# Axionis47/semantic-search-kd

Measured on AMD Instinct MI355X. Metric: docs embedded/sec + queries/sec@top-10 (1M×384-d corpus), 1→8 MI355X, higher is better.
Workload: dtype bf16 screen + f32 exact; 1 GPU; cosine top-10: 10000 queries x 1000000 x 384-d fp32 corpus in HBM (configs[1] search), row-sharded over 1 GPU(s), all-gather + merge; corpus_rows=1000000, queries=10000, k=10, queries_per_block=160, corpus_passes=63, slices=4, exact_fallback_queries=0, index_bytes=1536000000, sidecar_bytes=768004096, workspace_bytes=693437184

## Files before the change

### include/sskd_amd.h

```cpp
#ifndef SSKD_AMD_H
#define SSKD_AMD_H

#include <stddef.h>
#include <stdint.h>

#ifdef __cplusplus
extern "C" {
#endif

#define SSKD_ABI_VERSION 1

#define SSKD_OK 0
#define SSKD_ERR_INVALID 1
#define SSKD_ERR_WORKSPACE 2
#define SSKD_ERR_HIP 3
#define SSKD_ERR_UNSUPPORTED 4

#define SSKD_DIM 384
#define SSKD_TILE_ROWS 32
#define SSKD_K_PASS 32
#define SSKD_K_MAX 1024

int sskd_abi_version(void);
const char* sskd_last_error(void);
int sskd_device_count(void);

int64_t sskd_index_padded_rows(int64_t n_rows);
size_t sskd_index_tiled_bytes(int64_t n_rows);

int sskd_index_add_rows(const float* d_rows, int64_t n_rows, int normalize,
                        float* d_tiled, int64_t dst_row0, void* stream);

int sskd_index_get_rows(const float* d_tiled, int64_t row0, int64_t n_rows,
                        float* d_rows, void* stream);

int sskd_l2_normalize_rows(float* d_x, int64_t n_rows, int dim, void* stream);

size_t sskd_index_search_workspace_bytes(int64_t n_rows, int nq, int k);
int sskd_index_search(const float* d_tiled, int64_t n_rows,
                      const float* d_queries, int nq, int k, int64_t id_offset,
                      float* d_out_scores, int64_t* d_out_ids,
                      void* d_workspace, size_t workspace_bytes, void* stream);

typedef struct sskd_search_tuning {
  int32_t queries_per_block;
  int32_t target_workgroups;
  int32_t pruning_pools;
} sskd_search_tuning;

size_t sskd_index_search_workspace_bytes_ex(int64_t n_rows, int nq, int k,
                                            const sskd_search_tuning* tuning);
int sskd_index_search_ex(const float* d_tiled, int64_t n_rows, const float* d_queries, int nq,
                         int k, int64_t id_offset, float* d_out_scores, int64_t* d_out_ids,
                         void* d_workspace, size_t workspace_bytes, void* stream,
                         const sskd_search_tuning* tuning, void* ev_scan_begin, void* ev_scan_end);

int sskd_index_search_profiled(const float* d_tiled, int64_t n_rows,
                               const float* d_queries, int nq, int k, int64_t id_offset,
                               float* d_out_scores, int64_t* d_out_ids,
                               void* d_workspace, size_t workspace_bytes, void* stream,
                               void* ev_scan_begin, void* ev_scan_end);

size_t sskd_index_bf16_bytes(int64_t n_rows);
int sskd_index_make_bf16(const float* d_tiled, int64_t n_rows, void* d_bf16, void* stream);
size_t sskd_index_search_screened_workspace_bytes(int64_t n_rows, int nq, int k);
int sskd_index_search_screened_plan(int64_t n_rows, int nq, int k, int* queries_per_block, int* corpus_passes,
                                    int* n_slices);
int sskd_index_search_screened(const float* d_tiled, const void* d_bf16, int64_t n_rows, const float* d_queries,
                               int nq, int k, int64_t id_offset, float* d_out_scores, int64_t* d_out_ids,
                               int* d_status, void* d_workspace, size_t workspace_bytes, void* stream,
                               void* ev_scan_begin, void* ev_scan_end);

size_t sskd_index_screen_band_scratch_bytes(int nq);
int sskd_index_screen_band(const void* d_bf16, int64_t n_rows, const float* d_queries, int nq, float* d_eps2_out,
                           void* d_scratch, size_t scratch_bytes, void* stream);

int sskd_index_search_screened_plan_claims(int64_t n_rows, int nq, int k, int* claims);
int sskd_index_search_screened_claim(const float* d_tiled, const void* d_bf16, int64_t n_rows, const float* d_queries,
                                     int nq, int k, int64_t id_offset, const uint32_t* d_row_mask, int claim,
                                     float* d_out_scores, int64_t* d_out_ids, int* d_status, void* d_workspace,
                                     size_t workspace_bytes, void* stream, void* ev_scan_begin, void* ev_scan_end);

size_t sskd_index_search_onepass_workspace_bytes(int64_t n_rows, int nq, int k);
int sskd_index_search_onepass(const float* d_tiled, int64_t n_rows, const float* d_queries, int nq,
                              int k, int64_t id_offset, float* d_out_scores, int64_t* d_out_ids,
                              int* d_inexact, void* d_workspace, size_t workspace_bytes,
                              void* stream);

int64_t sskd_row_mask_words(int64_t n_rows);
int sskd_row_mask_pack(const uint8_t* d_flags, int64_t n_rows, uint32_t* d_mask, void* stream);
int sskd_row_mask_update(uint32_t* d_mask, int64_t n_rows, const int64_t* d_rows, int64_t n_ids, int allow,
                         int* d_bad, void* stream);
int sskd_row_mask_and(const uint32_t* d_a, const uint32_t* d_b, int64_t n_rows, uint32_t* d_out, void* stream);
int sskd_row_mask_count(const uint32_t* d_mask, int64_t n_rows, int64_t* d_count, void* stream);

int sskd_index_search_filtered(const float* d_tiled, int64_t n_rows, const float* d_queries, int nq, int k,
                               int64_t id_offset, const uint32_t* d_row_mask, float* d_out_scores,
                               int64_t* d_out_ids, void* d_workspace, size_t workspace_bytes, void* stream,
                               const sskd_search_tuning* tuning, void* ev_scan_begin, void* ev_scan_end);
int sskd_index_search_screened_filtered(const float* d_tiled, const void* d_bf16, int64_t n_rows, const float* d_queries,
                                        int nq, int k, int64_t id_offset, const uint32_t* d_row_mask, float* d_out_scores,
                                        int64_t* d_out_ids, int* d_status, void* d_workspace, size_t workspace_bytes,
                                        void* stream, void* ev_scan_begin, void* ev_scan_end);
int sskd_index_search_onepass_filtered(const float* d_tiled, int64_t n_rows, const float* d_queries, int nq,
                                       int k, int64_t id_offset, const uint32_t* d_row_mask, float* d_out_scores,
                                       int64_t* d_out_ids, int* d_inexact, void* d_workspace,
                                       size_t workspace_bytes, void* stream);

size_t sskd_index_range_search_workspace_bytes(int64_t n_rows, int nq, int64_t max_results);
int sskd_index_range_search(const float* d_tiled, int64_t n_rows, const float* d_queries, int nq,
                            const float* d_thresholds, int64_t id_offset, const uint32_t* d_row_mask, int64_t* d_lims,
                            float* d_out_scores, int64_t* d_out_ids, int64_t max_results, void* d_workspace,
                            size_t workspace_bytes, void* stream);

size_t sskd_range_record_bytes(int nq, int64_t cap);
size_t sskd_range_merge_workspace_bytes(int n_runs, int nq, int64_t max_results);
int sskd_range_merge_packed(const void* d_records, int n_runs, int nq, int64_t cap, int64_t* d_lims,
                            float* d_out_scores, int64_t* d_out_ids, int64_t max_results, void* d_workspace,
                            size_t workspace_bytes, void* stream);

size_t sskd_index_search_grouped_workspace_bytes(int64_t n_rows, int nq, int k, int k_rows);
int sskd_index_search_grouped(const float* d_tiled, int64_t n_rows, const float* d_queries, int nq, int k, int k_rows,
                              int64_t id_offset, const uint32_t* d_row_mask, const int32_t* d_row_group,
                              float* d_out_scores, int64_t* d_out_ids, int32_t* d_out_groups, int32_t* d_out_count,
                              int32_t* d_unproved, int32_t* d_n_unproved, void* d_workspace, size_t workspace_bytes,
                              void* stream);

int sskd_row_mask_rank(const uint32_t* d_mask, int64_t n_rows, int64_t* d_word_prefix, void* stream);
int sskd_index_compact_rows(const float* d_src_tiled, int64_t n_rows, const uint32_t* d_mask,
                            const int64_t* d_word_prefix, float* d_dst_tiled, void* stream);

int sskd_index_mine_select(const float* d_tiled, int64_t n_rows, const float* d_queries, int nq,
                           const float* d_rank_scores, const int64_t* d_rank_ids, int search_k,
                           const int64_t* d_pos_lims, const int32_t* d_pos_rows, const int32_t* d_row_groups,
                           double margin, int top_k, int64_t id_offset, float* d_out_scores, int64_t* d_out_ids,
                           int32_t* d_out_counts, float* d_out_max_pos, void* stream);

size_t sskd_bm25_search_workspace_bytes(int64_t n_rows, int nq, int k);
int sskd_bm25_search_plan(int64_t n_rows, int nq, int k, int* tile_rows, int* tiles, int* queries_per_chunk);
int sskd_bm25_search(const int64_t* d_term_offsets, const int32_t* d_post_rows, const double* d_post_w,
                     const double* d_idf, int64_t n_rows, int64_t n_terms, const int64_t* d_q_lims,
                     const int32_t* d_q_terms, int nq, int k, double* d_out_scores, int64_t* d_out_ids,
                     void* d_workspace, size_t workspace_bytes, void* stream);

int sskd_hybrid_fuse(const float* d_tiled, int64_t n_rows, const float* d_queries, const float* d_dense_scores,
                     const int64_t* d_dense_ids, int kd, const int64_t* d_term_offsets, const int32_t* d_post_rows,
                     const double* d_post_w, const double* d_idf, int64_t n_terms, const int64_t* d_q_lims,
                     const int32_t* d_q_terms, const double* d_bm25_scores, const int64_t* d_bm25_ids, int kb,
                     const uint32_t* d_mask, int method, double w_semantic, double w_bm25, double rrf_k, int nq, int k,
                     int64_t id_offset, double* d_out_scores, int64_t* d_out_ids, int32_t* d_out_counts,
                     float* d_out_dense, double* d_out_bm25, void* stream);

int sskd_eval_judge(const int64_t* d_rank_ids, int nq, int k_rank, int64_t id_offset, const int64_t* d_rel_lims,
                    const int32_t* d_rel_rows, const int32_t* d_rel_grades, int64_t n_rel, const double* d_discounts,
                    const int32_t* cutoffs, int n_cut, int ideal_mode, double* d_out_metrics, void* stream);
int sskd_eval_lists(const float* d_queries, const float* d_docs, int dim, const float* d_scores_in,
                    const int64_t* d_doc_lims, int64_t total, const int32_t* d_grades, const float* d_ref_scores,
                    const double* d_discounts, const int32_t* cutoffs, int n_cut, int ideal_mode, int nq,
                    double* d_out_metrics, float* d_out_scores, int32_t* d_out_order, int64_t* d_out_discordant,
                    void* stream);

int sskd_ivf_search_plan(int nq, int nprobe, int k, int64_t n_rows, int64_t max_list_rows, int* parts, int* chunk_rows,
                         int* workgroups);
size_t sskd_ivf_search_workspace_bytes(int nq, int nprobe, int k, int64_t n_rows, int64_t max_list_rows);
int sskd_ivf_search(const float* d_tiled, int64_t n_rows, const float* d_queries, int nq, const int64_t* d_probe,
                    int nprobe, const int64_t* d_list_offsets, const int32_t* d_list_rows, int nlist, int k,
                    int64_t id_offset, const uint32_t* d_row_mask, float* d_out_scores, int64_t* d_out_ids,
                    void* d_workspace, size_t workspace_bytes, void* stream);
int sskd_ivf_list_sums(const float* d_tiled, int64_t n_rows, const int64_t* d_list_offsets, const int32_t* d_list_rows,
                       int nlist, double* d_sums, void* stream);

int sskd_pq_encode(const float* d_rows, int64_t n, const float* d_centroids, const int64_t* d_assign, int nlist,
                   const float* d_codebooks, int m, uint8_t* d_codes, void* stream);
int sskd_pq_code_sums(const float* d_rows, int64_t n, const float* d_centroids, const int64_t* d_assign, int nlist,
                      const int64_t* d_group_offsets, const int32_t* d_group_rows, int m, double* d_sums,
                      int64_t* d_counts, void* stream);
int sskd_pq_lut(const float* d_queries, int nq, const float* d_codebooks, int m, float* d_lut, void* stream);
int sskd_pq_search_plan(int nq, int nprobe, int k, int refine, int m, int64_t n_rows, int64_t max_list_rows, int* parts,
                        int* min_part_rows, int* workgroups, size_t* lut_bytes);
size_t sskd_pq_search_workspace_bytes(int nq, int nprobe, int k, int refine, int m, int64_t n_rows,
                                      int64_t max_list_rows);
int sskd_pq_search(const float* d_tiled, int64_t n_rows, const float* d_queries, int nq, const int64_t* d_probe,
                   const float* d_probe_scores, int nprobe, const int64_t* d_list_offsets, const int32_t* d_list_rows,
                   int nlist, const uint8_t* d_codes_csr, const float* d_codebooks, int m, int k, int refine,
                   int64_t id_offset, const uint32_t* d_row_mask, float* d_out_scores, int64_t* d_out_ids,
                   int64_t* d_out_candidates, void* d_workspace, size_t workspace_bytes, void* stream);

int sskd_graph_prune(const int32_t* d_knn, int64_t n_rows, int knn_k, int M, int32_t* d_fwd, void* stream);
int sskd_graph_merge(const int32_t* d_fwd, const int32_t* d_rev, int64_t n_rows, int M, int32_t* d_graph, void* stream);
int sskd_graph_search_plan(int nq, int k, int ef, int width, int M, int n_seeds, int* workgroups, int* threads,
                           int* lds_bytes, int* step_rows);
size_t sskd_graph_search_workspace_bytes(int nq, int k, int ef, int width, int M, int n_seeds);
int sskd_graph_search(const float* d_tiled, int64_t n_rows, const int32_t* d_graph, int M, const float* d_queries, int nq,
                      const int64_t* d_seeds, int n_seeds, const int32_t* d_seed_rows, int64_t n_seed_rows, int k, int ef,
                      int width, int max_iterations, int64_t id_offset, const uint32_t* d_row_mask, float* d_out_scores,
                      int64_t* d_out_ids, int32_t* d_out_iterations, void* stream);

#define SSKD_LATE_TQ_MAX 128
#define SSKD_LATE_R_MAX 1024
int sskd_late_pack_tokens(const void* d_hidden, const int32_t* d_lengths, const int64_t* d_offsets, int B, int S,
                          int64_t n_tokens, void* d_tokens, void* stream);
int sskd_late_rerank_plan(int nq, int max_tq, int R, int k, int* workgroups, int* threads, int* lds_bytes, int* chunk);
size_t sskd_late_rerank_workspace_bytes(int nq, int R);
int sskd_late_rerank(const void* d_q_tokens, const int64_t* q_lims, const int64_t* d_q_lims, int nq, const void* d_tokens,
                     const int64_t* d_tok_lims, int64_t n_rows, int64_t n_tokens, const int64_t* d_candidates, int R, int k,
                     int64_t id_offset, float* d_out_scores, int64_t* d_out_ids, float* d_out_raw, void* d_workspace,
                     size_t workspace_bytes, void* stream);

#define SSKD_LATE_C_MAX 65536
int sskd_latec_compress(const void* d_tokens, const int64_t* d_assign, int64_t n, const void* d_centroids, int C,
                       const float* d_cutoffs, const float* d_weights, int nbits, int32_t* d_cid, float* d_scale,
                       uint8_t* d_codes, int64_t row0, int64_t n_store, void* stream);
int sskd_latec_rerank_plan(int nq, int max_tq, int R, int k, int nbits, int* workgroups, int* threads, int* lds_bytes,
                                     int* chunk);
size_t sskd_latec_rerank_workspace_bytes(int nq, int R);
int sskd_latec_rerank(const void* d_q_tokens, const int64_t* q_lims, const int64_t* d_q_lims, int nq,
                                const int32_t* d_cid, const float* d_scale, const uint8_t* d_codes, int nbits,
                                const void* d_centroids, int C, const float* d_weights, const int64_t* d_tok_lims, int64_t n_rows,
                                int64_t n_tokens, const int64_t* d_candidates, int R, int k, int64_t id_offset,
                                float* d_out_scores, int64_t* d_out_ids, float* d_out_raw, void* d_workspace,
                                size_t workspace_bytes, void* stream);

int sskd_kd_loss(const float* d_student, const float* d_teacher, int batch, int n_docs,
                 float temperature, float contrastive_temperature, float w_margin_mse,
                 float w_listwise, float w_contrastive, float* d_losses, float* d_grad,
                 float* d_row_workspace, void* stream);

int sskd_index_search_plan(int64_t n_rows, int nq, int k, int* queries_per_block,
                           int* corpus_passes, int* n_slices, int* waves_per_block,
                           int* scan_passes);

int sskd_index_search_plan_ex(int64_t n_rows, int nq, int k, const sskd_search_tuning* tuning,
                              int* queries_per_block, int* corpus_passes, int* n_slices,
                              int* waves_per_block, int* scan_passes);

int sskd_topk_merge(const float* d_scores, const int64_t* d_ids, int n_lists, int nq,
                    int k_in, int k_out, float* d_out_scores, int64_t* d_out_ids,
                    void* stream);

size_t sskd_topk_record_bytes(int nq, int k);
int sskd_topk_merge_packed(const void* d_records, int n_lists, int nq, int k_in, int k_out,
                           float* d_out_scores, int64_t* d_out_ids, void* stream);

int sskd_similarity(const float* d_q, int nq, const float* d_d, int nd, int dim,
                    float* d_out, void* stream);


int sskd_pool_normalize(const void* d_hidden, int hidden_is_bf16, const int32_t* d_mask,
                        int B, int S, int normalize, float* d_out, void* stream);

typedef struct sskd_encoder_config {
  int32_t vocab_size;
  int32_t hidden;
  int32_t layers;
  int32_t heads;
  int32_t intermediate;
  int32_t max_positions;
  int32_t type_vocab;
  float layer_norm_eps;
} sskd_encoder_config;

typedef struct sskd_encoder_layer_weights {
  const void* wqkv;
  const float* bqkv;
  const void* wo;
  const float* bo;
  const float* ln1_g;
  const float* ln1_b;
  const void* w1;
  const float* b1;
  const void* w2;
  const float* b2;
  const float* ln2_g;
  const float* ln2_b;
} sskd_encoder_layer_weights;

typedef struct sskd_encoder_weights {
  const void* word_emb;
  const void* pos_emb;
  const void* type_emb;
  const float* emb_ln_g;
  const float* emb_ln_b;
  const sskd_encoder_layer_weights* layers;
} sskd_encoder_weights;

size_t sskd_encoder_workspace_bytes(const sskd_encoder_config* cfg, int B, int S);

int sskd_encoder_forward(const sskd_encoder_config* cfg, const sskd_encoder_weights* w,
                         const int32_t* d_ids, const int32_t* d_mask, int B, int S,
                         int normalize, float* d_out, void* d_workspace,
                         size_t workspace_bytes, void* stream);

int sskd_encoder_hidden(const sskd_encoder_config* cfg, const sskd_encoder_weights* w,
                        const int32_t* d_ids, const int32_t* d_mask, int B, int S,
                        void* d_hidden_bf16, void* d_workspace, size_t workspace_bytes,
                        void* stream);

int sskd_encoder_probe(const sskd_encoder_config* cfg, const sskd_encoder_weights* w,
                       const int32_t* d_ids, const int32_t* d_mask, const int32_t* d_seg, int B, int S,
                       void* d_hidden_bf16, void* d_context_bf16, void* d_workspace,
                       size_t workspace_bytes, void* stream);


int sskd_pack_plan(const int32_t* lengths, int n_seq, int capacity, int32_t* table, int* n_rows);

int sskd_pack_tokens(const int32_t* d_flat_ids, const int32_t* d_cu_seqlens, const int32_t* d_table,
                     int n_seq, int n_rows, int capacity, int32_t* d_ids, int32_t* d_seg, void* stream);

int sskd_encoder_forward_packed(const sskd_encoder_config* cfg, const sskd_encoder_weights* w,
                                const int32_t* d_ids, const int32_t* d_seg, int n_rows, int capacity,
                                const int32_t* d_table, int n_seq, int normalize, float* d_out,
                                void* d_workspace, size_t workspace_bytes, void* stream);

typedef struct sskd_generic_config {
  int32_t vocab_size;
  int32_t hidden;
  int32_t layers;
  int32_t heads;
  int32_t intermediate;
  int32_t max_positions;
  int32_t type_vocab;
  float layer_norm_eps;
  int32_t pos_offset;
} sskd_generic_config;

typedef struct sskd_generic_layer_weights {
  const void* wqkv;
  const void* wqkv_t;
  const void* wo;
  const void* wo_t;
  const void* w1;
  const void* w1_t;
  const void* w2;
  const void* w2_t;
  const float* bqkv;
  const float* bo;
  const float* ln1_g;
  const float* ln1_b;
  const float* b1;
  const float* b2;
  const float* ln2_g;
  const float* ln2_b;
} sskd_generic_layer_weights;

typedef struct sskd_generic_weights {
  const void* word_emb;
  const void* pos_emb;
  const void* type_emb;
  const float* emb_ln_g;
  const float* emb_ln_b;
  const sskd_generic_layer_weights* layers;
} sskd_generic_weights;

typedef struct sskd_generic_layer_grads {
  float* wqkv;
  float* bqkv;
  float* wo;
  float* bo;
  float* ln1_g;
  float* ln1_b;
  float* w1;
  float* b1;
  float* w2;
  float* b2;
  float* ln2_g;
  float* ln2_b;
} sskd_generic_layer_grads;

typedef struct sskd_generic_grads {
  float* word_emb;
  float* pos_emb;
  float* type_emb;
  float* emb_ln_g;
  float* emb_ln_b;
  const sskd_generic_layer_grads* layers;
} sskd_generic_grads;

size_t sskd_generic_workspace_bytes(const sskd_generic_config* cfg, int B, int S, int training);

int sskd_generic_forward(const sskd_generic_config* cfg, const sskd_generic_weights* w, const int32_t* d_ids,
                         const int32_t* d_mask, int B, int S, int training, int pool, int normalize, void* d_out,
                         void* d_workspace, size_t workspace_bytes, void* stream);

int sskd_generic_backward(const sskd_generic_config* cfg, const sskd_generic_weights* w, const sskd_generic_grads* grads,
                          const int32_t* d_ids, const int32_t* d_mask, int B, int S, int normalize, const float* d_dout,
                          void* d_workspace, size_t workspace_bytes, void* stream);

size_t sskd_teacher_workspace_bytes(const sskd_generic_config* cfg, int B, int S);
int sskd_teacher_score(const sskd_generic_config* cfg, const sskd_generic_weights* w, const float* d_head_dense_w,
                       const float* d_head_dense_b, const float* d_head_out_w, const float* d_head_out_b,
                       const int32_t* d_ids, const int32_t* d_mask, int B, int S, float* d_logits, void* d_workspace,
                       size_t workspace_bytes, void* stream);

int sskd_gemm_nt_bf16(const void* d_a, const void* d_b, void* d_c, const float* d_bias, int M, int N, int K,
                      int c_is_f32, int accumulate, void* stream);
int sskd_gemm_backend(int mode);
int sskd_gemm_tn_bf16(const void* d_a, const void* d_b, float* d_c, int64_t T, int M, int N, void* stream);

typedef struct sskd_gemm_desc {
  const void* a;
  const void* b;
  void* c;
  const float* bias;
  int64_t lda, ldb, ldc;
  int64_t sa1, sa2, sb1, sb2, sc1, sc2;
  int32_t m, n, k;
  int32_t batch1, batch2;
  float alpha;
  int32_t c_is_f32;
  int32_t accumulate;
  int32_t split_k;
  int32_t act;
} sskd_gemm_desc;

int sskd_gemm_nt_ex(const sskd_gemm_desc* d, void* stream);

enum {
  SSKD_OP_ATTENTION_FWD = 1,
  SSKD_OP_ATTENTION_BWD = 2,
  SSKD_OP_SOFTMAX_FWD = 3,
  SSKD_OP_SOFTMAX_BWD = 4,
  SSKD_OP_ADD_LN_FWD = 5,
  SSKD_OP_LN_BWD = 6,
  SSKD_OP_GELU_FWD = 7,
  SSKD_OP_GELU_BWD = 8,
  SSKD_OP_GELU_BWD_COLSUM = 9,
  SSKD_OP_COLSUM = 10,
  SSKD_OP_ADD = 11,
  SSKD_OP_TRANSPOSE = 12,
  SSKD_OP_EMBED_FWD = 13,
  SSKD_OP_EMBED_BWD = 14,
  SSKD_OP_POOL_FWD = 15,
  SSKD_OP_POOL_BWD = 16,
  SSKD_OP_GEMM_TN = 17
};
int sskd_generic_op(int op, const void* const* ptrs, int n_ptrs, const int64_t* ints, int n_ints, const float* floats,
                    int n_floats, void* stream);


int sskd_tokenizer_create(const char* vocab_blob, int64_t blob_bytes, void** handle);
void sskd_tokenizer_destroy(void* handle);

int sskd_tokenizer_encode(void* handle, const char* text_blob, const int64_t* offsets, int n_texts,
                          int max_len, int n_threads, int32_t* out_ids, int64_t out_capacity,
                          int32_t* out_lengths, uint8_t* out_needs_unicode, int64_t* out_total);

#ifdef __cplusplus
}
#endif
#endif
```

### semantic-search-kd_amd/_native.py

```python
from __future__ import annotations

import ctypes as C
from pathlib import Path
from typing import Optional

_LIB_PATH = Path(__file__).resolve().parent / "libsskd_amd.so"

SSKD_OK = 0
SSKD_DIM = 384
SSKD_TILE_ROWS = 32
SSKD_K_PASS = 32
SSKD_K_MAX = 1024

_ERR_NAMES = {1: "INVALID", 2: "WORKSPACE", 3: "HIP", 4: "UNSUPPORTED"}


class NativeError(RuntimeError):

    def __init__(self, code: int, message: str):
        super().__init__(f"sskd_amd[{_ERR_NAMES.get(code, code)}]: {message}")
        self.code = code


class EncoderConfig(C.Structure):
    _fields_ = [
        ("vocab_size", C.c_int32),
        ("hidden", C.c_int32),
        ("layers", C.c_int32),
        ("heads", C.c_int32),
        ("intermediate", C.c_int32),
        ("max_positions", C.c_int32),
        ("type_vocab", C.c_int32),
        ("layer_norm_eps", C.c_float),
    ]


class EncoderLayerWeights(C.Structure):
    _fields_ = [
        (n, C.c_void_p)
        for n in ("wqkv", "bqkv", "wo", "bo", "ln1_g", "ln1_b", "w1", "b1", "w2", "b2", "ln2_g", "ln2_b")
    ]


class EncoderWeights(C.Structure):
    _fields_ = [
        ("word_emb", C.c_void_p),
        ("pos_emb", C.c_void_p),
        ("type_emb", C.c_void_p),
        ("emb_ln_g", C.c_void_p),
        ("emb_ln_b", C.c_void_p),
        ("layers", C.POINTER(EncoderLayerWeights)),
    ]


class GenericConfig(C.Structure):
    _fields_ = [
        ("vocab_size", C.c_int32), ("hidden", C.c_int32), ("layers", C.c_int32), ("heads", C.c_int32),
        ("intermediate", C.c_int32), ("max_positions", C.c_int32), ("type_vocab", C.c_int32),
        ("layer_norm_eps", C.c_float), ("pos_offset", C.c_int32),
    ]


GENERIC_LAYER_W = ("wqkv", "wqkv_t", "wo", "wo_t", "w1", "w1_t", "w2", "w2_t",
                   "bqkv", "bo", "ln1_g", "ln1_b", "b1", "b2", "ln2_g", "ln2_b")
GENERIC_LAYER_G = ("wqkv", "bqkv", "wo", "bo", "ln1_g", "ln1_b", "w1", "b1", "w2", "b2", "ln2_g", "ln2_b")


class GenericLayerWeights(C.Structure):
    _fields_ = [(n, C.c_void_p) for n in GENERIC_LAYER_W]


class GenericWeights(C.Structure):
    _fields_ = [(n, C.c_void_p) for n in ("word_emb", "pos_emb", "type_emb", "emb_ln_g", "emb_ln_b")] + [
        ("layers", C.POINTER(GenericLayerWeights))
    ]


class GenericLayerGrads(C.Structure):
    _fields_ = [(n, C.c_void_p) for n in GENERIC_LAYER_G]


class GenericGrads(C.Structure):
    _fields_ = [(n, C.c_void_p) for n in ("word_emb", "pos_emb", "type_emb", "emb_ln_g", "emb_ln_b")] + [
        ("layers", C.POINTER(GenericLayerGrads))
    ]


class GemmDesc(C.Structure):

    _fields_ = [("a", C.c_void_p), ("b", C.c_void_p), ("c", C.c_void_p), ("bias", C.c_void_p)] + [
        (n, C.c_int64) for n in ("lda", "ldb", "ldc", "sa1", "sa2", "sb1", "sb2", "sc1", "sc2")
    ] + [(n, C.c_int32) for n in ("m", "n", "k", "batch1", "batch2")] + [("alpha", C.c_float)] + [
        (n, C.c_int32) for n in ("c_is_f32", "accumulate", "split_k", "act")
    ]


OP_ATTENTION_FWD, OP_ATTENTION_BWD, OP_SOFTMAX_FWD, OP_SOFTMAX_BWD, OP_ADD_LN_FWD, OP_LN_BWD = 1, 2, 3, 4, 5, 6
OP_GELU_FWD, OP_GELU_BWD, OP_GELU_BWD_COLSUM, OP_COLSUM, OP_ADD, OP_TRANSPOSE = 7, 8, 9, 10, 11, 12
OP_EMBED_FWD, OP_EMBED_BWD, OP_POOL_FWD, OP_POOL_BWD, OP_GEMM_TN = 13, 14, 15, 16, 17


class SearchTuning(C.Structure):

    _fields_ = [("queries_per_block", C.c_int32), ("target_workgroups", C.c_int32), ("pruning_pools", C.c_int32)]


_vp, _i, _i64, _sz = C.c_void_p, C.c_int, C.c_int64, C.c_size_t
_ip = C.POINTER(C.c_int)
_f = C.c_float
SIGNATURES = {
    "sskd_abi_version": (_i, []),
    "sskd_last_error": (C.c_char_p, []),
    "sskd_device_count": (_i, []),
    "sskd_index_padded_rows": (_i64, [_i64]),
    "sskd_index_tiled_bytes": (_sz, [_i64]),
    "sskd_index_add_rows": (_i, [_vp, _i64, _i, _vp, _i64, _vp]),
    "sskd_index_get_rows": (_i, [_vp, _i64, _i64, _vp, _vp]),
    "sskd_l2_normalize_rows": (_i, [_vp, _i64, _i, _vp]),
    "sskd_index_search_workspace_bytes": (_sz, [_i64, _i, _i]),
    "sskd_index_search": (_i, [_vp, _i64, _vp, _i, _i, _i64, _vp, _vp, _vp, _sz, _vp]),
    "sskd_index_search_profiled": (_i, [_vp, _i64, _vp, _i, _i, _i64, _vp, _vp, _vp, _sz, _vp, _vp, _vp]),
    "sskd_index_search_plan": (_i, [_i64, _i, _i, _ip, _ip, _ip, _ip, _ip]),
    "sskd_index_search_workspace_bytes_ex": (_sz, [_i64, _i, _i, C.POINTER(SearchTuning)]),
    "sskd_index_search_ex": (
        _i, [_vp, _i64, _vp, _i, _i, _i64, _vp, _vp, _vp, _sz, _vp, C.POINTER(SearchTuning), _vp, _vp]
    ),
    "sskd_index_search_plan_ex": (_i, [_i64, _i, _i, C.POINTER(SearchTuning), _ip, _ip, _ip, _ip, _ip]),
    "sskd_topk_record_bytes": (_sz, [_i, _i]),
    "sskd_topk_merge_packed": (_i, [_vp, _i, _i, _i, _i, _vp, _vp, _vp]),
    "sskd_index_bf16_bytes": (_sz, [_i64]),
    "sskd_index_make_bf16": (_i, [_vp, _i64, _vp, _vp]),
    "sskd_index_search_screened_workspace_bytes": (_sz, [_i64, _i, _i]),
    "sskd_index_search_screened_plan": (_i, [_i64, _i, _i, _ip, _ip, _ip]),
    "sskd_index_search_screened": (_i, [_vp, _vp, _i64, _vp, _i, _i, _i64, _vp, _vp, _vp, _vp, _sz, _vp, _vp, _vp]),
    "sskd_index_search_screened_plan_claims": (_i, [_i64, _i, _i, _ip]),
    "sskd_index_search_screened_claim": (
        _i, [_vp, _vp, _i64, _vp, _i, _i, _i64, _vp, _i, _vp, _vp, _vp, _vp, _sz, _vp, _vp, _vp]
    ),
    "sskd_index_screen_band_scratch_bytes": (_sz, [_i]),
    "sskd_index_screen_band": (_i, [_vp, _i64, _vp, _i, _vp, _vp, _sz, _vp]),
    "sskd_index_search_onepass_workspace_bytes": (_sz, [_i64, _i, _i]),
    "sskd_index_search_onepass": (_i, [_vp, _i64, _vp, _i, _i, _i64, _vp, _vp, _vp, _vp, _sz, _vp]),
    "sskd_row_mask_words": (_i64, [_i64]),
    "sskd_row_mask_pack": (_i, [_vp, _i64, _vp, _vp]),
    "sskd_row_mask_update": (_i, [_vp, _i64, _vp, _i64, _i, _vp, _vp]),
    "sskd_row_mask_and": (_i, [_vp, _vp, _i64, _vp, _vp]),
    "sskd_row_mask_count": (_i, [_vp, _i64, _vp, _vp]),
    "sskd_index_search_filtered": (
        _i, [_vp, _i64, _vp, _i, _i, _i64, _vp, _vp, _vp, _vp, _sz, _vp, C.POINTER(SearchTuning), _vp, _vp]
    ),
    "sskd_index_search_screened_filtered": (
        _i, [_vp, _vp, _i64, _vp, _i, _i, _i64, _vp, _vp, _vp, _vp, _vp, _sz, _vp, _vp, _vp]
    ),
    "sskd_index_search_onepass_filtered": (_i, [_vp, _i64, _vp, _i, _i, _i64, _vp, _vp, _vp, _vp, _vp, _sz, _vp]),
    "sskd_index_range_search_workspace_bytes": (_sz, [_i64, _i, _i64]),
    "sskd_index_range_search": (_i, [_vp, _i64, _vp, _i, _vp, _i64, _vp, _vp, _vp, _vp, _i64, _vp, _sz, _vp]),
    "sskd_range_record_bytes": (_sz, [_i, _i64]),
    "sskd_range_merge_workspace_bytes": (_sz, [_i, _i, _i64]),
    "sskd_range_merge_packed": (_i, [_vp, _i, _i, _i64, _vp, _vp, _vp, _i64, _vp, _sz, _vp]),
    "sskd_index_search_grouped_workspace_bytes": (_sz, [_i64, _i, _i, _i]),
    "sskd_index_search_grouped": (
        _i, [_vp, _i64, _vp, _i, _i, _i, _i64, _vp, _vp, _vp, _vp, _vp, _vp, _vp, _vp, _vp, _sz, _vp]
    ),
    "sskd_row_mask_rank": (_i, [_vp, _i64, _vp, _vp]),
    "sskd_index_compact_rows": (_i, [_vp, _i64, _vp, _vp, _vp, _vp]),
    "sskd_index_mine_select": (
        _i, [_vp, _i64, _vp, _i, _vp, _vp, _i, _vp, _vp, _vp, C.c_double, _i, _i64, _vp, _vp, _vp, _vp, _vp]
    ),
    "sskd_bm25_search_workspace_bytes": (_sz, [_i64, _i, _i]),
    "sskd_bm25_search_plan": (_i, [_i64, _i, _i, _ip, _ip, _ip]),
    "sskd_bm25_search": (_i, [_vp, _vp, _vp, _vp, _i64, _i64, _vp, _vp, _i, _i, _vp, _vp, _vp, _sz, _vp]),
    "sskd_hybrid_fuse": (
        _i, [_vp, _i64, _vp, _vp, _vp, _i, _vp, _vp, _vp, _vp, _i64, _vp, _vp, _vp, _vp, _i, _vp, _i, C.c_double,
             C.c_double, C.c_double, _i, _i, _i64, _vp, _vp, _vp, _vp, _vp, _vp]
    ),
    "sskd_eval_judge": (_i, [_vp, _i, _i, _i64, _vp, _vp, _vp, _i64, _vp, _vp, _i, _i, _vp, _vp]),
    "sskd_eval_lists": (
        _i, [_vp, _vp, _i, _vp, _vp, _i64, _vp, _vp, _vp, _vp, _i, _i, _i, _vp, _vp, _vp, _vp, _vp]
    ),
    "sskd_ivf_search_plan": (_i, [_i, _i, _i, _i64, _i64, _ip, _ip, _ip]),
    "sskd_ivf_search_workspace_bytes": (_sz, [_i, _i, _i, _i64, _i64]),
    "sskd_ivf_search": (_i, [_vp, _i64, _vp, _i, _vp, _i, _vp, _vp, _i, _i, _i64, _vp, _vp, _vp, _vp, _sz, _vp]),
    "sskd_ivf_list_sums": (_i, [_vp, _i64, _vp, _vp, _i, _vp, _vp]),
    "sskd_pq_encode": (_i, [_vp, _i64, _vp, _vp, _i, _vp, _i, _vp, _vp]),
    "sskd_pq_code_sums": (_i, [_vp, _i64, _vp, _vp, _i, _vp, _vp, _i, _vp, _vp, _vp]),
    "sskd_pq_lut": (_i, [_vp, _i, _vp, _i, _vp, _vp]),
    "sskd_pq_search_plan": (_i, [_i, _i, _i, _i, _i, _i64, _i64, _ip, _ip, _ip, C.POINTER(_sz)]),
    "sskd_pq_search_workspace_bytes": (_sz, [_i, _i, _i, _i, _i, _i64, _i64]),
    "sskd_pq_search": (
        _i, [_vp, _i64, _vp, _i, _vp, _vp, _i, _vp, _vp, _i, _vp, _vp, _i, _i, _i, _i64, _vp, _vp, _vp, _vp, _vp, _sz, _vp]
    ),
    "sskd_graph_prune": (_i, [_vp, _i64, _i, _i, _vp, _vp]),
    "sskd_graph_merge": (_i, [_vp, _vp, _i64, _i, _vp, _vp]),
    "sskd_graph_search_plan": (_i, [_i, _i, _i, _i, _i, _i, _ip, _ip, _ip, _ip]),
    "sskd_graph_search_workspace_bytes": (_sz, [_i, _i, _i, _i, _i, _i]),
    "sskd_graph_search": (
        _i, [_vp, _i64, _vp, _i, _vp, _i, _vp, _i, _vp, _i64, _i, _i, _i, _i, _i64, _vp, _vp, _vp, _vp, _vp]
    ),
    "sskd_late_pack_tokens": (_i, [_vp, _vp, _vp, _i, _i, _i64, _vp, _vp]),
    "sskd_late_rerank_plan": (_i, [_i, _i, _i, _i, _ip, _ip, _ip, _ip]),
    "sskd_late_rerank_workspace_bytes": (_sz, [_i, _i]),
    "sskd_late_rerank": (
        _i, [_vp, _vp, _vp, _i, _vp, _vp, _i64, _i64, _vp, _i, _i, _i64, _vp, _vp, _vp, _vp, _sz, _vp]
    ),
    "sskd_latec_compress": (_i, [_vp, _vp, _i64, _vp, _i, _vp, _vp, _i, _vp, _vp, _vp, _i64, _i64, _vp]),
    "sskd_latec_rerank_plan": (_i, [_i, _i, _i, _i, _i, _ip, _ip, _ip, _ip]),
    "sskd_latec_rerank_workspace_bytes": (_sz, [_i, _i]),
    "sskd_latec_rerank": (
        _i, [_vp, _vp, _vp, _i, _vp, _vp, _vp, _i, _vp, _i, _vp, _vp, _i64, _i64, _vp, _i, _i, _i64, _vp, _vp, _vp, _vp, _sz, _vp]
    ),
    "sskd_topk_merge": (_i, [_vp, _vp, _i, _i, _i, _i, _vp, _vp, _vp]),
    "sskd_kd_loss": (_i, [_vp, _vp, _i, _i, _f, _f, _f, _f, _f, _vp, _vp, _vp, _vp]),
    "sskd_similarity": (_i, [_vp, _i, _vp, _i, _i, _vp, _vp]),
    "sskd_pool_normalize": (_i, [_vp, _i, _vp, _i, _i, _i, _vp, _vp]),
    "sskd_encoder_workspace_bytes": (_sz, [C.POINTER(EncoderConfig), _i, _i]),
    "sskd_encoder_forward": (
        _i,
        [C.POINTER(EncoderConfig), C.POINTER(EncoderWeights), _vp, _vp, _i, _i, _i, _vp, _vp, _sz, _vp],
    ),
    "sskd_pack_plan": (_i, [_vp, _i, _i, _vp, _ip]),
    "sskd_pack_tokens": (_i, [_vp, _vp, _vp, _i, _i, _i, _vp, _vp, _vp]),
    "sskd_encoder_forward_packed": (
        _i,
        [C.POINTER(EncoderConfig), C.POINTER(EncoderWeights), _vp, _vp, _i, _i, _vp, _i, _i, _vp, _vp, _sz, _vp],
    ),
    "sskd_generic_workspace_bytes": (_sz, [C.POINTER(GenericConfig), _i, _i, _i]),
    "sskd_generic_forward": (
        _i, [C.POINTER(GenericConfig), C.POINTER(GenericWeights), _vp, _vp, _i, _i, _i, _i, _i, _vp, _vp, _sz, _vp]
    ),
    "sskd_generic_backward": (
        _i, [C.POINTER(GenericConfig), C.POINTER(GenericWeights), C.POINTER(GenericGrads), _vp, _vp, _i, _i, _i, _vp,
             _vp, _sz, _vp]
    ),
    "sskd_teacher_workspace_bytes": (_sz, [C.POINTER(GenericConfig), _i, _i]),
    "sskd_teacher_score": (
        _i, [C.POINTER(GenericConfig), C.POINTER(GenericWeights), _vp, _vp, _vp, _vp, _vp, _vp, _i, _i, _vp, _vp, _sz, _vp]
    ),
    "sskd_gemm_nt_bf16": (_i, [_vp, _vp, _vp, _vp, _i, _i, _i, _i, _i, _vp]),
    "sskd_gemm_backend": (_i, [_i]),
    "sskd_gemm_tn_bf16": (_i, [_vp, _vp, _vp, _i64, _i, _i, _vp]),
    "sskd_gemm_nt_ex": (_i, [C.POINTER(GemmDesc), _vp]),
    "sskd_generic_op": (_i, [_i, C.POINTER(_vp), _i, C.POINTER(_i64), _i, C.POINTER(_f), _i, _vp]),
    "sskd_tokenizer_create": (_i, [C.c_char_p, _i64, C.POINTER(C.c_void_p)]),
    "sskd_tokenizer_destroy": (None, [_vp]),
    "sskd_tokenizer_encode": (_i, [_vp, C.c_char_p, _vp, _i, _i, _i, _vp, _i64, _vp, _vp, C.POINTER(_i64)]),
    "sskd_encoder_hidden": (
        _i,
        [C.POINTER(EncoderConfig), C.POINTER(EncoderWeights), _vp, _vp, _i, _i, _vp, _vp, _sz, _vp],
    ),
    "sskd_encoder_probe": (
        _i,
        [C.POINTER(EncoderConfig), C.POINTER(EncoderWeights), _vp, _vp, _vp, _i, _i, _vp, _vp, _vp, _sz, _vp],
    ),
}

_lib: Optional[C.CDLL] = None


def lib_path() -> Path:
    return _LIB_PATH


def load() -> C.CDLL:
    global _lib
    if _lib is not None:
        return _lib
    if not _LIB_PATH.exists():
        raise ImportError(
            f"{_LIB_PATH} is missing: the MI355X HIP extension is not built. "
            "Run `python -c 'import __graft_entry__ as g; g.build()'` (needs hipcc). "
            "There is no CPU fallback."
        )
    lib = C.CDLL(str(_LIB_PATH))
    for name, (res, args) in SIGNATURES.items():
        fn = getattr(lib, name)
        fn.restype = res
        fn.argtypes = args
    _lib = lib
    return lib


def check(code: int) -> None:
    if code != SSKD_OK:
        msg = load().sskd_last_error()
        raise NativeError(code, msg.decode("utf-8", "replace") if msg else "unknown error")


def require_gpu() -> None:
    import torch

    if not torch.cuda.is_available():
        raise RuntimeError(
            "semantic-search-kd_amd is an MI355X-only backend: no HIP device is visible "
            "(torch.cuda.is_available() is False) and there is no CPU path."
        )
    load()


def current_stream_ptr(device=None) -> int:
    import torch

    return int(torch.cuda.current_stream(device).cuda_stream)


def grown(buf, need_bytes: int, device):
    import torch

    if buf is not None and buf.numel() >= need_bytes:
        return buf
    return torch.empty(max(int(need_bytes), 1), dtype=torch.uint8, device=device)


def as_device_i32(x, device):
    import numpy as np
    import torch

    t = x if isinstance(x, torch.Tensor) else torch.from_numpy(np.ascontiguousarray(np.asarray(x)))
    return t.to(device=device, dtype=torch.int32)


def padded_ids_mask(input_ids, attention_mask, device, pad_id: int = 0):
    import torch

    ids = as_device_i32(input_ids, device)
    mask = torch.ones_like(ids) if attention_mask is None else as_device_i32(attention_mask, device)
    S = ids.shape[1]
    Sp = max(32, -(-S // 32) * 32)
    if Sp != S:
        ids = torch.nn.functional.pad(ids, (0, Sp - S), value=pad_id)
        mask = torch.nn.functional.pad(mask, (0, Sp - S))
    return ids.contiguous(), mask.contiguous()
```

### semantic-search-kd_amd/csrc/screen.hip

```cpp
#include "search_device.h"
#include "search_host.h"

#include <algorithm>
#include <cfloat>

using sskd::require_shard_rows;

namespace {

typedef __bf16 sbf16x8 __attribute__((ext_vector_type(8)));
constexpr int BSTEPS = DIM / 16;
constexpr int BTILE_VEC = BSTEPS * 64;
#ifndef SSKD_SCREEN_BGROUP
#define SSKD_SCREEN_BGROUP 6
#endif
#ifndef SSKD_SCREEN_WAVES
#define SSKD_SCREEN_WAVES 12
#endif
#ifndef SSKD_SCREEN_RING
#define SSKD_SCREEN_RING 2
#endif
constexpr int BGROUP = SSKD_SCREEN_BGROUP;
constexpr int SCREEN_RING = SSKD_SCREEN_RING;
constexpr int BGROUP_Q5 = 3, SCREEN_RING_Q5 = 2;
#ifndef SSKD_SCREEN_TAU_REFRESH_TILES
#define SSKD_SCREEN_TAU_REFRESH_TILES 64
#endif
constexpr int SCREEN_TAU_REFRESH_TILES = SSKD_SCREEN_TAU_REFRESH_TILES;
constexpr int SCREEN_WAVES = SSKD_SCREEN_WAVES;
template <int BG, int RG>
struct ScreenRingOk {
  static_assert(BSTEPS % BG == 0 && (BSTEPS / BG) % RG == 0 && RG >= 2, "screening prefetch geometry");
  static constexpr bool value = true;
};
static_assert(ScreenRingOk<BGROUP, SCREEN_RING>::value && ScreenRingOk<BGROUP_Q5, SCREEN_RING_Q5>::value, "");
constexpr float SCREEN_ACC_SLACK = 1.0e-4f;
constexpr int SCREEN_MAX_CAND = 256;
constexpr int SCREEN_FALLBACK_TIER1 = 1024;
constexpr int SCREEN_LIGHT_MAX_TILES_PER_WAVE = 330;
constexpr int SCREEN_CUS = 256;

__global__ __launch_bounds__(256) void tile_colsum_kernel(const float4* __restrict__ tiled, int64_t n_tiles,
                                                          float* __restrict__ colsum) {
  const int c = threadIdx.x % CHUNKS, g = threadIdx.x / CHUNKS;
  if (g >= 2) return;
  float4 a = make_float4(0.f, 0.f, 0.f, 0.f);
  for (int64_t t = blockIdx.x; t < n_tiles; t += gridDim.x) {
    const float4* src = tiled + t * (int64_t)(TILE_ROWS * CHUNKS);
#pragma unroll 4
    for (int r = g; r < TILE_ROWS; r += 2) {
      const float4 v = src[r * CHUNKS + c];
      a.x += v.x; a.y += v.y; a.z += v.z; a.w += v.w;
    }
  }
  atomicAdd(colsum + 4 * c + 0, a.x); atomicAdd(colsum + 4 * c + 1, a.y);
  atomicAdd(colsum + 4 * c + 2, a.z); atomicAdd(colsum + 4 * c + 3, a.w);
}

constexpr int SIDECAR_NORM_BYTES = 4096;
constexpr int SIDECAR_ABSMAX_WORD = 3;
constexpr int SIDECAR_COLSUM_OFF = 64;

__global__ __launch_bounds__(256) void make_bf16_tiles_kernel(const float4* __restrict__ tiled, int64_t n_tiles, int64_t n_rows,
                                                              sbf16x8* __restrict__ out, int* __restrict__ norm_block) {
  __shared__ float rowss[3][32];
  __shared__ float mu[DIM];
  __shared__ int amax;
  const int64_t t = blockIdx.x;
  if (threadIdx.x < 96) rowss[threadIdx.x >> 5][threadIdx.x & 31] = 0.f;
  if (threadIdx.x == 0) amax = 0;
  const float inv_n = 1.0f / (float)n_rows;
  for (int c = threadIdx.x; c < DIM; c += 256) mu[c] = reinterpret_cast<const float*>(norm_block)[SIDECAR_COLSUM_OFF + c] * inv_n;
  __syncthreads();
  const float4* src = tiled + t * (int64_t)(TILE_ROWS * CHUNKS);
  for (int v = threadIdx.x; v < BTILE_VEC; v += 256) {
    const int sidx = v >> 6, l = v & 63, r = l & 31, hh = l >> 5;
    const int u = 2 * sidx + hh;
    const float4 a = src[tile_idx4(r, 2 * u)], b = src[tile_idx4(r, 2 * u + 1)];
    const float x[8] = {a.x, a.y, a.z, a.w, b.x, b.y, b.z, b.w};
    const bool live = t * TILE_ROWS + r < n_rows;
    sbf16x8 o;
    float nn = 0.f, bb = 0.f, dd = 0.f;
    int am = 0;
#pragma unroll
    for (int e = 0; e < 8; ++e) {
      const float xc = live ? x[e] - mu[8 * u + e] : 0.f;
      o[e] = (__bf16)xc;
      const float xr = (float)o[e];
      const float d = xr - xc;
      am = max(am, __float_as_int(x[e]) & 0x7fffffff);
      nn = fmaf(x[e], x[e], nn);
      bb = fmaf(xr, xr, bb);
      dd = fmaf(d, d, dd);
    }
    out[t * BTILE_VEC + v] = o;
    atomicAdd(&rowss[0][r], nn);
    atomicAdd(&rowss[1][r], bb);
    atomicAdd(&rowss[2][r], dd);
    atomicMax(&amax, am);
  }
  __syncthreads();
  if (threadIdx.x < 96) {
    const float v = rowss[threadIdx.x >> 5][threadIdx.x & 31];
    atomicMax(norm_block + (threadIdx.x >> 5), __float_as_int(v < INFINITY ? v : INFINITY));
  }
  if (threadIdx.x == 96) atomicMax(norm_block + SIDECAR_ABSMAX_WORD, amax);
}

constexpr float SCREEN_MIN_CORPUS = 0x1p-40f, SCREEN_MIN_QUERY = 0x1p-96f;
constexpr float SCREEN_MIN_BAND = 0x1p-100f, SCREEN_MAX_BAND = 0x1p+100f;
__global__ __launch_bounds__(256) void screen_setup_kernel(const float* __restrict__ queries, int nq,
                                                           const int* __restrict__ max_norm2, float* __restrict__ eps2,
                                                           int* __restrict__ tau, int* __restrict__ fb_count,
                                                           int* __restrict__ d_status, int* __restrict__ cursors,
                                                           int n_cursors) {
  for (int i = blockIdx.x * 256 + threadIdx.x; i < n_cursors; i += gridDim.x * 256) cursors[i] = 0;
  if (threadIdx.x < 44) {
    const int64_t i = (int64_t)blockIdx.x * 44 + threadIdx.x;
    if (i < (int64_t)nq * 11) tau[i] = (int)0x80000000;
  }
  if (blockIdx.x == 0) {
    if (threadIdx.x < 64) fb_count[threadIdx.x] = 0;
    if (threadIdx.x < 2) d_status[threadIdx.x] = 0;
  }
  const int lane = threadIdx.x & 63;
  const int q = blockIdx.x * 4 + (threadIdx.x >> 6);
  if (q >= nq) return;
  float xs[DIM / 64];
  int am = 0;
#pragma unroll
  for (int i = 0; i < DIM / 64; ++i) {
    xs[i] = queries[(int64_t)q * DIM + lane + 64 * i];
    am = max(am, __float_as_int(xs[i]) & 0x7fffffff);
  }
#pragma unroll
  for (int o = 32; o > 0; o >>= 1) am = max(am, __shfl_xor(am, o));
  const int ex = min(max(am >> 23, 1), 253);
  const float down = __int_as_float(ex << 23), up = __int_as_float((254 - ex) << 23);
  float ss = 0.f, dd = 0.f;
#pragma unroll
  for (int i = 0; i < DIM / 64; ++i) {
    const float x = xs[i];
    const float d = ((float)(__bf16)x - x) * up;
    const float xu = x * up;
    ss = fmaf(xu, xu, ss);
    dd = fmaf(d, d, dd);
  }
  ss = wave_sum(ss);
  dd = wave_sum(dd);
  if (lane == 0) {
    const float cn = sqrtf(__int_as_float(max_norm2[0])), cb = sqrtf(__int_as_float(max_norm2[1])),
                cd = sqrtf(__int_as_float(max_norm2[2]));
    const float ca = __int_as_float(max_norm2[SIDECAR_ABSMAX_WORD]), qa = __int_as_float(am);
    const float qn = sqrtf(ss), qd = sqrtf(dd);
    const float band = 2.0f * (qd * cb + qn * cd + SCREEN_ACC_SLACK * qn * fmaxf(cn, cb)) * 1.0002f * down;
    const bool zero = (qa == 0.f || ca == 0.f) && band == 0.f;
    const bool sound = zero || (qa >= SCREEN_MIN_QUERY && ca >= SCREEN_MIN_CORPUS && ca < INFINITY &&
                                band >= SCREEN_MIN_BAND && band <= SCREEN_MAX_BAND);
    eps2[q] = sound ? band + 1e-30f : INFINITY;
  }
}

template <int BG>
__device__ __forceinline__ void load_bgroup(sbf16x8 (&buf)[BG], const sbf16x8* __restrict__ base, unsigned lane_off) {
  asm volatile("" : "+v"(lane_off));
#pragma unroll
  for (int s = 0; s < BG; ++s)
    buf[s] = *reinterpret_cast<const sbf16x8*>(reinterpret_cast<const char*>(base + s * 64) + lane_off);
}

typedef __attribute__((address_space(3))) const sbf16x8 screen_lds_frag;
constexpr int SCREEN_FRAGS_PER_BASE = 64;
template <int QB>
constexpr int screen_frag_bases() { return (QB * BSTEPS + SCREEN_FRAGS_PER_BASE - 1) / SCREEN_FRAGS_PER_BASE; }
#ifndef SSKD_SCREEN_FRAG_DEPTH
#define SSKD_SCREEN_FRAG_DEPTH 2
#endif
constexpr int SCREEN_FRAG_DEPTH = SSKD_SCREEN_FRAG_DEPTH;
static_assert(SCREEN_FRAG_DEPTH >= 2, "the fragment ring holds the MFMA's own operand and at least one read ahead");

template <int QB, int NB>
__device__ __forceinline__ sbf16x8 read_qfrag(screen_lds_frag* const (&qbase)[NB], int I) {
  const int f = (I % QB) * BSTEPS + I / QB;
  return qbase[f / SCREEN_FRAGS_PER_BASE][(f % SCREEN_FRAGS_PER_BASE) * 64];
}

template <int QB, int G, int BG, int D, int NB>
__device__ __forceinline__ void compute_bgroup(const sbf16x8 (&a)[BG], screen_lds_frag* const (&qbase)[NB], sbf16x8 (&b)[D],
                                               f32x16 (&acc)[QB]) {
  constexpr int N = BG * QB, I0 = G * N, TOTAL = BSTEPS * QB;
  asm volatile("" ::: "memory");
#ifndef SSKD_SCREEN_ABL_NOLDS
  if constexpr (G == 0) {
#pragma unroll
    for (int i = 0; i < D - 1; ++i) b[i % D] = read_qfrag<QB>(qbase, i);
  }
#endif
#pragma unroll
  for (int i = 0; i < N; ++i) {
    const int I = I0 + i, s = i / QB, qq = i % QB;
#ifdef SSKD_SCREEN_ABL_NOLDS
    const sbf16x8 bi = a[(s + qq) % BG];
#else
    if (I + D - 1 < TOTAL) b[(I + D - 1) % D] = read_qfrag<QB>(qbase, I + D - 1);
    const sbf16x8 bi = b[I % D];
#endif
    __builtin_amdgcn_sched_barrier(0);
    acc[qq] = __builtin_amdgcn_mfma_f32_32x32x16_bf16(a[s], bi, acc[qq], 0, 0, 0);
    __builtin_amdgcn_sched_barrier(0);
  }
}

template <int QB, int G, int BG, int RG, int D, int NB>
__device__ __forceinline__ void screen_tile_groups(sbf16x8 (&buf)[RG][BG], const sbf16x8* __restrict__ tile,
                                                   screen_lds_frag* const (&qbase)[NB], sbf16x8 (&b)[D], f32x16 (&acc)[QB],
                                                   bool more, int64_t next_tile, unsigned lane_off) {
  constexpr int NG = BSTEPS / BG;
  if constexpr (G < NG) {
    constexpr int PG = G + RG - 1;
#ifndef SSKD_SCREEN_ABL_NOGLOBAL
    if constexpr (PG < NG) load_bgroup<BG>(buf[PG % RG], tile + PG * BG * 64, lane_off);
    else if (more) load_bgroup<BG>(buf[PG % RG], tile + next_tile + (PG - NG) * BG * 64, lane_off);
#endif
    compute_bgroup<QB, G, BG, D, NB>(buf[G % RG], qbase, b, acc);
    screen_tile_groups<QB, G + 1, BG, RG, D, NB>(buf, tile, qbase, b, acc, more, next_tile, lane_off);
  }
}

#ifndef SSKD_SCREEN_CAP
#define SSKD_SCREEN_CAP 64
#endif
#ifndef SSKD_SCREEN_FIN_ENTRIES
#define SSKD_SCREEN_FIN_ENTRIES 640
#endif
constexpr int SCREEN_CAP = SSKD_SCREEN_CAP;
#ifndef SSKD_SCREEN_PRE_TILES
#define SSKD_SCREEN_PRE_TILES 64
#endif
constexpr int SCREEN_PRE_TILES = SSKD_SCREEN_PRE_TILES;
constexpr int SCREEN_FIN_ENTRIES = SSKD_SCREEN_FIN_ENTRIES;
static_assert(SCREEN_FIN_ENTRIES >= 640, "the streaming path of the finalize kernel parks 64 x 10 scores in the stage");

#ifndef SSKD_SCREEN_CLAIM_TILES
#define SSKD_SCREEN_CLAIM_TILES 8
#endif
constexpr int SCREEN_CLAIM_TILES = SSKD_SCREEN_CLAIM_TILES;
#ifndef SSKD_SCREEN_CLAIM_MIN_CHUNKS
#define SSKD_SCREEN_CLAIM_MIN_CHUNKS 2
#endif
#ifndef SSKD_SCREEN_CLAIM_MIN_QBLOCKS
#define SSKD_SCREEN_CLAIM_MIN_QBLOCKS 32
#endif
constexpr int SCREEN_CLAIM_MIN_CHUNKS = SSKD_SCREEN_CLAIM_MIN_CHUNKS, SCREEN_CLAIM_MIN_QBLOCKS = SSKD_SCREEN_CLAIM_MIN_QBLOCKS;
static_assert(SCREEN_CLAIM_TILES >= 2, "the claim for the next chunk is issued one whole tile before the chunk in hand ends");
#ifdef SSKD_SCREEN_NO_STEAL
constexpr bool SCREEN_STEAL = false;
#else
constexpr bool SCREEN_STEAL = true;
#endif

struct ScreenAppendParams {
  const sbf16x8* tiled;
  const float* queries;
  const float* eps2;
  uint2* cand;
  int* cand_cnt;
  int* tau;
  int* gpool;
  int* cursors;
  int64_t n_rows;
  int n_tiles;
  int nq;
  int n_slices;
  int tiles_per_slice;
  int lists_per_query;
  int pre_tiles;
  int pre_tps;
  int claim;
  const uint32_t* row_mask;
#ifdef SSKD_SCREEN_STAMPS
  unsigned long long* stamps;
#endif
};

__device__ __attribute__((noinline)) int screen_compact_run(unsigned long long* run, int n, float thr) {
  int w = 0;
  for (int i = 0; i < n; ++i) {
    const unsigned long long e = __hip_atomic_load(run + i, __ATOMIC_RELAXED, __HIP_MEMORY_SCOPE_AGENT);
    if (__uint_as_float((unsigned)e) >= thr) run[w++] = e;
  }
  return w;
}

template <int K, int QB, int WAVES, bool BOUND_ONLY, bool LIGHT, int BG, int RG, bool MASKED = false>
__device__ __forceinline__ void screen_tiles(const ScreenAppendParams& p, int t_begin, int t_end, int slice, int* cursors,
                                             int wave, int j, int h, int q0,
                                             const sbf16x8* __restrict__ qlane,
                                             int* __restrict__ pool, int* __restrict__ wthr, uint2* run0, int64_t run_stride,
                                             bool ragged, float (&gthr)[QB], const float (&band)[QB], int (&cnt)[QB]) {
  sbf16x8 buf[RG][BG];
  constexpr int NB = screen_frag_bases<QB>();
  screen_lds_frag* qbase[NB];
#pragma unroll
  for (int nb = 0; nb < NB; ++nb) {
    qbase[nb] = (screen_lds_frag*)qlane + nb * SCREEN_FRAGS_PER_BASE * 64;
    asm volatile("" : "+v"(qbase[nb]));
  }
  sbf16x8 qfrag[SCREEN_FRAG_DEPTH];
  const unsigned lane_off = (unsigned)(j + 32 * h) * 16u;
  int n_real = p.nq - q0 - j;
  asm volatile("" : "+v"(n_real));
  constexpr int CH = SCREEN_CLAIM_TILES;
  int t, next_t, c_end = 0, next_end = 0, sl = slice, s_begin = t_begin, s_end = t_end, left = p.n_slices - 1, drawn = 0;
  bool in_flight = false;
  const auto draw = [&]() {
    drawn = 0;
    int at = sl;
    asm volatile("" : "+v"(at));
    if (j + 32 * h == 0) drawn = __hip_atomic_fetch_add(cursors + at, 1, __ATOMIC_RELAXED, __HIP_MEMORY_SCOPE_AGENT);
    in_flight = true;
  };
  const auto drawn_chunk = [&]() -> int {
    for (;;) {
      if (!in_flight) draw();
      in_flight = false;
      const int c = __builtin_amdgcn_readfirstlane(drawn);
      const int nt = s_begin + (c + WAVES) * CH;
      if (nt < s_end) {
        next_end = min(nt + CH, s_end);
        return nt;
      }
      if (!SCREEN_STEAL || left == 0) return -1;
      --left;
      sl = sl + 1 == p.n_slices ? 0 : sl + 1;
      s_begin = sl * p.tiles_per_slice;
      s_end = min(s_begin + p.tiles_per_slice, p.n_tiles);
    }
  };
  const bool dealt = BOUND_ONLY || !p.claim;
  if (dealt) {
    t = t_begin + wave < t_end ? t_begin + wave : -1;
  } else {
    t = t_begin + wave * CH;
    c_end = min(t + CH, t_end);
    if (t >= t_end) {
      t = drawn_chunk();
      c_end = next_end;
    }
  }
  if (t >= 0) {
#pragma unroll
    for (int g = 0; g + 1 < RG; ++g) load_bgroup<BG>(buf[g], p.tiled + (int64_t)t * BTILE_VEC + g * BG * 64, lane_off);
  }

  for (int tiles_done = 0; t >= 0; t = next_t, ++tiles_done) {
    if (dealt) {
      next_t = t + WAVES < t_end ? t + WAVES : -1;
    } else {
      const int rem = c_end - t;
      if (rem == 2) draw();
      next_t = t + 1;
      if (rem == 1) {
        next_t = drawn_chunk();
        c_end = next_end;
      }
    }
    const sbf16x8* tile = p.tiled + (int64_t)t * BTILE_VEC;
    uint32_t mword = 0xFFFFFFFFu;
    if constexpr (MASKED) mword = tile_mask_word(p.row_mask, t);
    const bool exchange = !BOUND_ONLY && (tiles_done == 0 || tiles_done == 16 || tiles_done % SCREEN_TAU_REFRESH_TILES == 0);
#pragma unroll
    for (int qq = 0; qq < QB; ++qq) {
      const int w = wthr[qq * 32 + j];
      gthr[qq] = fmaxf(gthr[qq], ordered_to_float(w) - band[qq]);
      if (exchange && (qq * 32 < n_real))
        gthr[qq] = fmaxf(gthr[qq],
                         ordered_to_float(exchange_bound<K>(p.gpool, p.tau + q0 + qq * 32 + j, q0 + qq * 32 + j, w)) - band[qq]);
    }
    f32x16 acc[QB];
#pragma unroll
    for (int qq = 0; qq < QB; ++qq)
#pragma unroll
      for (int r = 0; r < 16; ++r) acc[qq][r] = 0.f;

    screen_tile_groups<QB, 0, BG, RG, SCREEN_FRAG_DEPTH, NB>(buf, tile, qbase, qfrag, acc, next_t >= 0,
                                                             BOUND_ONLY ? (int64_t)WAVES * BTILE_VEC
                                                                        : (int64_t)(next_t - t) * BTILE_VEC, lane_off);

    const int rowbase = t * TILE_ROWS + 4 * h;
    if (ragged && (int64_t)(t + 1) * TILE_ROWS > p.n_rows) {
#pragma unroll
      for (int qq = 0; qq < QB; ++qq)
#pragma unroll
        for (int r = 0; r < 16; ++r)
          if (rowbase + acc_row(r) >= p.n_rows) acc[qq][r] = -INFINITY;
    }
    if constexpr (MASKED) apply_tile_mask<QB>(acc, mword, h);
#ifdef SSKD_SCREEN_ABL_NOLIST
#pragma unroll
    for (int qq = 0; qq < QB; ++qq)
#pragma unroll
      for (int r = 0; r < 16; ++r) asm volatile("" ::"v"(acc[qq][r]));
    if (false)
#endif
#pragma unroll
    for (int qq = 0; qq < QB; ++qq) {
      float m = acc[qq][0];
#pragma unroll
      for (int r = 1; r < 16; ++r) m = fmaxf(m, acc[qq][r]);
      if constexpr (BOUND_ONLY) {
        if ((qq * 32 < n_real) && m >= gthr[qq]) {
          int xid = rowbase;
#pragma unroll
          for (int r = 15; r >= 0; --r) xid = acc[qq][r] == m ? rowbase + acc_row(r) : xid;
          const int xi = float_to_ordered(m);
          if (pool_offer<K>(pool + (qq * 32 + j) * K, wthr + qq * 32 + j, xi)) {
            int qa = q0 + qq * 32 + j;
            asm volatile("" : "+v"(qa));
            bucket_forward<K>(p.gpool, qa, xid, xi);
          }
          gthr[qq] = fmaxf(gthr[qq], ordered_to_float(wthr[qq * 32 + j]) - band[qq]);
        }
      } else
      if (__any((qq * 32 < n_real) && m >= gthr[qq])) {
#ifndef SSKD_SCREEN_NO_COMPACT
        {
          const bool tight = cnt[qq] > SCREEN_CAP - 16 && cnt[qq] <= SCREEN_CAP;
          if (__any(tight)) {
            __builtin_amdgcn_s_waitcnt(0x0F70);
            if (tight) cnt[qq] = screen_compact_run(reinterpret_cast<unsigned long long*>(run0 + qq * run_stride), cnt[qq], gthr[qq]);
          }
        }
#endif
        bool grew = false;
#pragma unroll
        for (int r = 0; r < 16; ++r) {
          const float x = acc[qq][r];
          const int xid = rowbase + acc_row(r);
          const bool take = (qq * 32 < n_real) && x >= gthr[qq];
          {
            if (take) {
              {
                unsigned long long* const run = reinterpret_cast<unsigned long long*>(run0 + qq * run_stride);
                if (cnt[qq] < SCREEN_CAP)
                  run[cnt[qq]] = (unsigned long long)__float_as_uint(x) | ((unsigned long long)(unsigned)xid << 32);
                ++cnt[qq];
              }
              if (!LIGHT && tiles_done > 0) {
                const int xi = float_to_ordered(x);
                if (pool_offer<K>(pool + (qq * 32 + j) * K, wthr + qq * 32 + j, xi) && (qq * 32 < n_real))
                  bucket_forward<K>(p.gpool, q0 + qq * 32 + j, xid, xi);
              }
              grew = true;
            }
          }
        }
        if (grew) {
          if constexpr (LIGHT) {
            int xid = rowbase;
#pragma unroll
            for (int r = 15; r >= 0; --r) xid = acc[qq][r] == m ? rowbase + acc_row(r) : xid;
            const int xi = float_to_ordered(m);
            if (pool_offer<K>(pool + (qq * 32 + j) * K, wthr + qq * 32 + j, xi) && tiles_done > 0)
              bucket_forward<K>(p.gpool, q0 + qq * 32 + j, xid, xi);
          } else {
            if (tiles_done == 0) pool_offer<K>(pool + (qq * 32 + j) * K, wthr + qq * 32 + j, float_to_ordered(m));
          }
          gthr[qq] = fmaxf(gthr[qq], ordered_to_float(wthr[qq * 32 + j]) - band[qq]);
        }
      }
    }
  }

}

template <int K, int QB, int WAVES, bool LIGHT, int BG, int RG, bool MASKED = false>
__global__ __launch_bounds__(WAVES * 64) void screen_append_kernel(ScreenAppendParams p) {
  extern __shared__ float4 qs_raw[];
  sbf16x8* const qs = reinterpret_cast<sbf16x8*>(qs_raw);
  const int tid = threadIdx.x;
  const int lane = tid & 63;
  const int wave = __builtin_amdgcn_readfirstlane(tid >> 6);
  const int j = lane & 31, h = lane >> 5;
  const int n_qblocks = gridDim.x / p.n_slices;
  const int xcd = blockIdx.x & 7, within = blockIdx.x >> 3;
  const int logical = xcd * (gridDim.x >> 3) + min(xcd, (int)(gridDim.x & 7)) + within;
  const int slice = logical / n_qblocks;
  const int qblk = logical % n_qblocks;
  const int q0 = qblk * (32 * QB);
#ifdef SSKD_SCREEN_STAMPS
  unsigned long long* const stamp = p.stamps + ((int64_t)blockIdx.x * WAVES + wave) * 3;
  if (lane == 0) stamp[0] = __builtin_amdgcn_s_memrealtime();
#endif

  for (int idx = tid; idx < QB * BSTEPS * 64; idx += WAVES * 64) {
    const int l = idx & 63, sidx = (idx >> 6) % BSTEPS, qq = idx / (64 * BSTEPS);
    const int q = q0 + qq * 32 + (l & 31);
    sbf16x8 v;
#pragma unroll
    for (int e = 0; e < 8; ++e) v[e] = (__bf16)0.f;
    if (q < p.nq) {
      const float4* src = reinterpret_cast<const float4*>(p.queries + (int64_t)q * DIM + 16 * sidx + 8 * (l >> 5));
      const float4 a = src[0], b = src[1];
      v[0] = (__bf16)a.x; v[1] = (__bf16)a.y; v[2] = (__bf16)a.z; v[3] = (__bf16)a.w;
      v[4] = (__bf16)b.x; v[5] = (__bf16)b.y; v[6] = (__bf16)b.z; v[7] = (__bf16)b.w;
    }
    qs[idx] = v;
  }
  int* const pool = reinterpret_cast<int*>(qs + QB * BSTEPS * 64);
  int* const wthr = pool + QB * 32 * K;
  for (int i = tid; i < QB * 32 * (K + 1); i += WAVES * 64) pool[i] = (int)0x80000000;
  __syncthreads();
  const sbf16x8* qlane = qs + lane;

  float gthr[QB];
  float band[QB];
  int cnt[QB];
  bool real[QB];
#pragma unroll
  for (int qq = 0; qq < QB; ++qq) {
    gthr[qq] = -FLT_MAX;
    const int qg = q0 + qq * 32 + j;
    real[qq] = qg < p.nq;
    band[qq] = p.eps2[real[qq] ? qg : p.nq - 1];
    cnt[qq] = 0;
  }
  const int my_list = (slice * WAVES + wave) * 2 + h;
  uint2* const run0 = p.cand + ((int64_t)min(q0 + j, p.nq - 1) * p.lists_per_query + my_list) * SCREEN_CAP;
  const int64_t run_stride = (int64_t)32 * p.lists_per_query * SCREEN_CAP;

  const bool ragged = (p.n_rows & 31) != 0;

  const int t_begin = slice * p.tiles_per_slice;
  const int t_end = min(t_begin + p.tiles_per_slice, p.n_tiles);
  if (p.pre_tps > 0) {
    const int s_begin = slice * p.pre_tps;
    const int s_end = min(s_begin + p.pre_tps, p.pre_tiles);
    screen_tiles<K, QB, WAVES, true, LIGHT, BG, RG, MASKED>(p, s_begin, s_end, slice, nullptr, wave, j, h, q0, qlane,
                                             pool, wthr, run0, run_stride, ragged, gthr, band, cnt);
#pragma unroll
    for (int qq = 0; qq < QB; ++qq)
      if (real[qq] && h == 0) atomicMax(p.tau + q0 + qq * 32 + j, wthr[qq * 32 + j]);
    __syncthreads();
    if ((SCREEN_STEAL && p.claim) || (s_begin < t_end && t_begin < s_end)) {
      for (int i = tid; i < QB * 32 * K; i += WAVES * 64) pool[i] = (int)0x80000000;
      __syncthreads();
    }
  }
#ifdef SSKD_SCREEN_STAMPS
  if (lane == 0) stamp[1] = __builtin_amdgcn_s_memrealtime();
#endif
  screen_tiles<K, QB, WAVES, false, LIGHT, BG, RG, MASKED>(p, t_begin, t_end, slice, p.cursors + (int64_t)qblk * p.n_slices,
                                            wave, j, h, q0, qlane, pool, wthr, run0, run_stride, ragged, gthr, band, cnt);
#ifdef SSKD_SCREEN_STAMPS
  if (lane == 0) stamp[2] = __builtin_amdgcn_s_memrealtime();
#endif

  int jt = j;
  asm volatile("" : "+v"(jt));
#pragma unroll
  for (int qq = 0; qq < QB; ++qq) {
    const int q = q0 + qq * 32 + jt;
    if (q < p.nq) p.cand_cnt[(int64_t)q * p.lists_per_query + my_list] = cnt[qq];
  }
}

struct ScreenFinalAppendParams {
  const uint2* cand;
  const int* cand_cnt;
  const float* eps2;
  const float* rows;
  const float* queries;
  int lists, k, nq;
  int64_t id_offset;
  float* out_scores;
  int64_t* out_ids;
  int* fb_count;
  int* fb_qid;
  float* fb_queries;
};

__global__ __launch_bounds__(64) void screen_finalize_append_kernel(ScreenFinalAppendParams p) {
  extern __shared__ __attribute__((aligned(16))) float fin_lds[];
  float* const es = fin_lds;
  int* const ei = reinterpret_cast<int*>(fin_lds + SCREEN_FIN_ENTRIES);
  float* const qv = fin_lds + 2 * SCREEN_FIN_ENTRIES;
  int* const ci = reinterpret_cast<int*>(qv + DIM);
  const int q = blockIdx.x, lane = threadIdx.x;
  for (int c = lane; c < DIM; c += 64) qv[c] = p.queries[(int64_t)q * DIM + c];

  bool bad = !(p.eps2[q] < INFINITY);
  int total = 0;
  for (int l0 = 0; l0 < p.lists; l0 += 64) {
    const int l = l0 + lane;
    const int c = l < p.lists ? p.cand_cnt[(int64_t)q * p.lists + l] : 0;
    if (c > SCREEN_CAP) bad = true;
    total += wave_sum(min(c, SCREEN_CAP));
  }
  int M = 0;
  float tau;
  if (total <= SCREEN_FIN_ENTRIES) {
    int base = 0;
    for (int l0 = 0; l0 < p.lists; l0 += 64) {
      const int l = l0 + lane;
      const int c = l < p.lists ? min(p.cand_cnt[(int64_t)q * p.lists + l], SCREEN_CAP) : 0;
      int incl = c;
#pragma unroll
      for (int o = 1; o < 64; o <<= 1) {
        const int v = __shfl_up(incl, o);
        if (lane >= o) incl += v;
      }
      const int off = base + incl - c;
      const uint2* src = p.cand + ((int64_t)q * p.lists + l) * SCREEN_CAP;
      for (int i = 0; i < c; ++i) {
        const uint2 e = src[i];
        es[off + i] = __uint_as_float(e.x);
        ei[off + i] = (int)e.y;
      }
      base += __shfl(incl, 63);
    }
    const int L = total;
    __builtin_amdgcn_s_waitcnt(0xC07F);

    float bs = INFINITY;
    int bi = -1;
    bool have = false;
    float kth = -INFINITY;
    int found = 0;
    for (int r = 0; r < p.k; ++r) {
      float s = -INFINITY;
      int i = -1;
      for (int e = lane; e < L; e += 64) {
        pick_after(s, i, es[e], ei[e], have, bs, bi);
      }
      wave_argbest(s, i);
      if (i < 0) break;
      bs = s; bi = i; have = true;
      kth = s;
      ++found;
    }
    tau = found == p.k ? kth - p.eps2[q] : -INFINITY;

    for (int e0 = 0; e0 < L; e0 += 64) {
      const int e = e0 + lane;
      const bool in = e < L && es[e] >= tau;
      const unsigned long long mask = __ballot(in);
      if (in) {
        const int slot = M + __popcll(mask & ((1ull << lane) - 1ull));
        if (slot < SCREEN_MAX_CAND) ci[slot] = ei[e];
      }
      M += __popcll(mask);
    }
  } else {
    float top[10];
#pragma unroll
    for (int i = 0; i < 10; ++i) top[i] = -INFINITY;
    for (int l = lane; l < p.lists; l += 64) {
      const int c = min(p.cand_cnt[(int64_t)q * p.lists + l], SCREEN_CAP);
      const uint2* src = p.cand + ((int64_t)q * p.lists + l) * SCREEN_CAP;
      for (int i = 0; i < c; ++i) {
        float v = __uint_as_float(src[i].x);
        if (v > top[9]) {
          top[9] = v;
#pragma unroll
          for (int u = 9; u > 0; --u) {
            const float a = top[u - 1], b = top[u];
            top[u - 1] = fmaxf(a, b);
            top[u] = fminf(a, b);
          }
        }
      }
    }
#pragma unroll
    for (int i = 0; i < 10; ++i) {
      es[lane * 10 + i] = top[i];
      ei[lane * 10 + i] = top[i] > -INFINITY ? lane * 10 + i : -1;
    }
    __builtin_amdgcn_s_waitcnt(0xC07F);
    float bs = INFINITY;
    int bi = -1;
    bool have = false;
    float kth = -INFINITY;
    int found = 0;
    for (int r = 0; r < p.k; ++r) {
      float s = -INFINITY;
      int i = -1;
      for (int e = lane; e < 640; e += 64) {
        const int id = ei[e];
        if (id >= 0) pick_after(s, i, es[e], id, have, bs, bi);
      }
      wave_argbest(s, i);
      if (i < 0) break;
      bs = s; bi = i; have = true;
      kth = s;
      ++found;
    }
    tau = found == p.k ? kth - p.eps2[q] : -INFINITY;
    int* const mcount = ei;
    __builtin_amdgcn_s_waitcnt(0xC07F);
    if (lane == 0) mcount[0] = 0;
    __builtin_amdgcn_s_waitcnt(0xC07F);
    for (int l = lane; l < p.lists; l += 64) {
      const int c = min(p.cand_cnt[(int64_t)q * p.lists + l], SCREEN_CAP);
      const uint2* src = p.cand + ((int64_t)q * p.lists + l) * SCREEN_CAP;
      for (int i = 0; i < c; ++i) {
        const uint2 e = src[i];
        if (__uint_as_float(e.x) >= tau) {
          const int slot = atomicAdd(mcount, 1);
          if (slot < SCREEN_MAX_CAND) ci[slot] = (int)e.y;
        }
      }
    }
    __builtin_amdgcn_s_waitcnt(0xC07F);
    M = mcount[0];
  }
  if (M > SCREEN_MAX_CAND) bad = true;
  if (__any(bad)) {
    int slot = 0;
    if (lane == 0) {
      slot = atomicAdd(p.fb_count, 1);
      p.fb_qid[slot] = q;
    }
    slot = __shfl(slot, 0);
    for (int c = lane; c < DIM; c += 64) p.fb_queries[(int64_t)slot * DIM + c] = qv[c];
    return;
  }
  __builtin_amdgcn_s_waitcnt(0xC07F);

  float cs[SCREEN_MAX_CAND / 64];
  int cid[SCREEN_MAX_CAND / 64];
#pragma unroll
  for (int c = 0; c < SCREEN_MAX_CAND / 64; ++c) {
    cs[c] = -INFINITY;
    cid[c] = -1;
    const int idx = c * 64 + lane;
    if (idx < M) {
      const int row = ci[idx];
      const float4* src = reinterpret_cast<const float4*>(p.rows) + (int64_t)row * (DIM / 4);
      float acc = 0.f;
#pragma unroll 16
      for (int u = 0; u < STEPS; ++u) {
        const float4 a = src[2 * u], b = src[2 * u + 1];
        const float4 qa = *reinterpret_cast<const float4*>(&qv[8 * u]), qb = *reinterpret_cast<const float4*>(&qv[8 * u + 4]);
        acc = fmaf(a.x, qa.x, acc); acc = fmaf(b.x, qb.x, acc);
        acc = fmaf(a.y, qa.y, acc); acc = fmaf(b.y, qb.y, acc);
        acc = fmaf(a.z, qa.z, acc); acc = fmaf(b.z, qb.z, acc);
        acc = fmaf(a.w, qa.w, acc); acc = fmaf(b.w, qb.w, acc);
      }
      cs[c] = acc;
      cid[c] = (acc == acc) ? row : -1;
    }
  }
  float bs = INFINITY;
  int bi = -1;
  bool have = false;
  for (int r = 0; r < p.k; ++r) {
    float s = -INFINITY;
    int i = -1;
#pragma unroll
    for (int c = 0; c < SCREEN_MAX_CAND / 64; ++c) {
      if (cid[c] >= 0) pick_after(s, i, cs[c], cid[c], have, bs, bi);
    }
    wave_argbest(s, i);
    if (lane == 0) {
      p.out_scores[(int64_t)q * p.k + r] = i >= 0 ? s : -FLT_MAX;
      p.out_ids[(int64_t)q * p.k + r] = i >= 0 ? (int64_t)i + p.id_offset : -1;
    }
    if (i < 0) {
      for (int rr = r + 1 + lane; rr < p.k; rr += 64) {
        p.out_scores[(int64_t)q * p.k + rr] = -FLT_MAX;
        p.out_ids[(int64_t)q * p.k + rr] = -1;
      }
      break;
    }
    bs = s; bi = i; have = true;
  }
}

__global__ void screen_fallback_tiers_kernel(int* __restrict__ fb_count, int tier1) {
  const int n = fb_count[0];
  fb_count[1] = n < tier1 ? n : tier1;
  fb_count[2] = n > tier1 ? n - tier1 : 0;
}

__global__ __launch_bounds__(256) void screen_scatter_kernel(const int* __restrict__ fb_count, const int* __restrict__ fb_qid,
                                                             const float* __restrict__ fb_scores,
                                                             const int64_t* __restrict__ fb_ids, int k,
                                                             float* __restrict__ out_scores, int64_t* __restrict__ out_ids,
                                                             int* __restrict__ d_status) {
  const int n = *fb_count;
  if (blockIdx.x == 0 && threadIdx.x == 0) d_status[1] = n;
  for (int i = blockIdx.x; i < n; i += gridDim.x) {
    const int q = fb_qid[i];
    for (int r = threadIdx.x; r < k; r += 256) {
      out_scores[(int64_t)q * k + r] = fb_scores[(int64_t)i * k + r];
      out_ids[(int64_t)q * k + r] = fb_ids[(int64_t)i * k + r];
    }
  }
}

}

extern "C" {


namespace {
struct ScreenPlan {
  int QB, LK, n_qblocks, n_slices, tiles_per_slice, n_tiles, lists_per_query;
  int pre_tiles, pre_slices, pre_tps;
  bool light;
  bool claim;
  size_t part_elems;
};

bool screen_plan(int64_t n_rows, int nq, int k, ScreenPlan* sp) {
  if (k < 1 || k > 10 || nq < 64 || n_rows < 64 * TILE_ROWS) return false;
  ScreenPlan pl{};
  pl.n_tiles = (int)sskd::ceil_div(n_rows, TILE_ROWS);
  const int resident = SCREEN_CUS;
  const int max_slices = std::max(1, (int)sskd::ceil_div(pl.n_tiles, SCREEN_WAVES));
  const double matrix_ms = (double)n_rows * nq * (2.0 * DIM) / 1.0e12;
  const double warm_ms = 0.09 * nq / 10000.0;
  int slices = 1;
  double best = 1e300;
  for (int qb : {4, 5, 2}) {
    if (qb == 2 ? nq >= 256 : nq < 256) continue;
#ifdef SSKD_SCREEN_FORCE_QB
    if (qb != SSKD_SCREEN_FORCE_QB) continue;
#endif
    const int qblocks = (int)sskd::ceil_div(nq, 32 * qb);
    for (int rounds = 1; rounds <= 8; ++rounds) {
      const int sl = std::min(std::max(1, rounds * resident / qblocks), max_slices);
      const int wgs = sl * qblocks;
      const double util = (double)wgs / ((double)resident * sskd::ceil_div(wgs, resident));
      const double cost = matrix_ms / util + warm_ms * sl;
      if (cost < best - 1e-9) { best = cost; slices = sl; pl.QB = qb; }
    }
  }
  if (pl.QB == 0) return false;
  pl.n_qblocks = (int)sskd::ceil_div(nq, 32 * pl.QB);
  pl.LK = SCREEN_CAP;
  const int max_by_lists = 1024 / (2 * SCREEN_WAVES);
  if (slices > max_by_lists) slices = max_by_lists;
#ifdef SSKD_SCREEN_FORCE_SLICES
  slices = SSKD_SCREEN_FORCE_SLICES;
#endif
  pl.tiles_per_slice = (int)sskd::ceil_div(pl.n_tiles, slices);
  pl.n_slices = (int)sskd::ceil_div(pl.n_tiles, pl.tiles_per_slice);
  pl.lists_per_query = pl.n_slices * SCREEN_WAVES * 2;
  pl.part_elems = (size_t)nq * pl.lists_per_query * pl.LK;
  pl.light = pl.tiles_per_slice <= SCREEN_LIGHT_MAX_TILES_PER_WAVE * SCREEN_WAVES;
  pl.claim = pl.tiles_per_slice >= SCREEN_CLAIM_MIN_CHUNKS * SCREEN_WAVES * SCREEN_CLAIM_TILES &&
             pl.n_qblocks >= SCREEN_CLAIM_MIN_QBLOCKS;
  pl.pre_tiles = std::min(SCREEN_PRE_TILES, pl.n_tiles / 8);
  pl.pre_slices = pl.n_slices;
  pl.pre_tps = (int)sskd::ceil_div(pl.pre_tiles, pl.n_slices);
  *sp = pl;
  return true;
}

struct ScreenWs {
  float* part_scores;
  int* part_ids;
  int* cand_cnt;
  int* tau;
  float* eps2;
  int* fb_count;
  int* cursors;
  int* fb_qid;
  float* fb_queries;
  float* fb_scores;
  int64_t* fb_ids;
  void* exact_ws;
  size_t exact_bytes;
  void* exact_ws2;
  size_t exact_bytes2;
#ifdef SSKD_SCREEN_STAMPS
  unsigned long long* stamps;
#endif
  size_t bytes;
};

ScreenWs screen_carve(void* base, const ScreenPlan& pl, int64_t n_rows, int nq, int k) {
  sskd::Carver c(base);
  ScreenWs w{};
  w.part_scores = c.take<float>(pl.part_elems);
  w.part_ids = c.take<int>(pl.part_elems);
  w.cand_cnt = c.take<int>((size_t)nq * pl.lists_per_query);
  w.tau = c.take<int>((size_t)nq * 11);
  w.eps2 = c.take<float>(nq);
  w.fb_count = c.take<int>(64);
  w.cursors = c.take<int>((size_t)pl.n_qblocks * pl.n_slices);
  w.fb_qid = c.take<int>(nq);
  w.fb_queries = c.take<float>((size_t)nq * DIM);
  w.fb_scores = c.take<float>((size_t)nq * k);
  w.fb_ids = c.take<int64_t>((size_t)nq * k);
  const int tier1 = nq < SCREEN_FALLBACK_TIER1 ? nq : SCREEN_FALLBACK_TIER1;
  w.exact_bytes = sskd::exact_workspace_bytes(n_rows, tier1, k);
  w.exact_ws = c.take<char>(w.exact_bytes);
  w.exact_bytes2 = nq > tier1 ? sskd::exact_workspace_bytes(n_rows, nq - tier1, k) : 0;
  w.exact_ws2 = w.exact_bytes2 ? c.take<char>(w.exact_bytes2) : nullptr;
#ifdef SSKD_SCREEN_STAMPS
  w.stamps = c.take<unsigned long long>((size_t)pl.n_qblocks * pl.n_slices * SCREEN_WAVES * 3);
#endif
  w.bytes = c.bytes();
  return w;
}
}

static inline size_t sidecar_norm_offset(int64_t n_rows) { return (size_t)sskd::ceil_div(n_rows, TILE_ROWS) * BTILE_VEC * 16; }
static inline size_t sidecar_rows_offset(int64_t n_rows) { return sidecar_norm_offset(n_rows) + SIDECAR_NORM_BYTES; }

static inline void launch_screen_setup(const int* max_norm2, const float* d_queries, int nq, float* eps2, int* tau,
                                       int* fb_count, int* d_status, int* cursors, int n_cursors, hipStream_t st) {
  hipLaunchKernelGGL(screen_setup_kernel, dim3((unsigned)sskd::ceil_div(nq, 4)), dim3(256), 0, st, d_queries, nq, max_norm2,
                     eps2, tau, fb_count, d_status, cursors, n_cursors);
}

size_t sskd_index_bf16_bytes(int64_t n_rows) {
  if (n_rows <= 0) return 0;
  return sidecar_rows_offset(n_rows);
}

int sskd_index_make_bf16(const float* d_tiled, int64_t n_rows, void* d_bf16, void* stream) {
  SSKD_REQUIRE(n_rows >= 0, "index_make_bf16: n_rows < 0");
  if (n_rows == 0) return SSKD_OK;
  SSKD_REQUIRE(d_tiled && d_bf16, "index_make_bf16: null pointer");
  hipStream_t st = sskd::as_stream(stream);
  const int64_t tiles = sskd::ceil_div(n_rows, TILE_ROWS);
  int* max_norm2 = reinterpret_cast<int*>(static_cast<char*>(d_bf16) + sidecar_norm_offset(n_rows));
  if (hipMemsetAsync(max_norm2, 0, SIDECAR_NORM_BYTES, st) != hipSuccess) return sskd::fail(SSKD_ERR_HIP, "index_make_bf16: memset failed");
  hipLaunchKernelGGL(tile_colsum_kernel, dim3((unsigned)(tiles < 1024 ? tiles : 1024)), dim3(256), 0, st,
                     reinterpret_cast<const float4*>(d_tiled), tiles, reinterpret_cast<float*>(max_norm2) + SIDECAR_COLSUM_OFF);
  int rc = sskd::check_launch("tile_colsum_kernel");
  if (rc != SSKD_OK) return rc;
  hipLaunchKernelGGL(make_bf16_tiles_kernel, dim3((unsigned)tiles), dim3(256), 0, st,
                     reinterpret_cast<const float4*>(d_tiled), tiles, n_rows, static_cast<sbf16x8*>(d_bf16), max_norm2);
  return sskd::check_launch("make_bf16_tiles_kernel");
}

size_t sskd_index_screen_band_scratch_bytes(int nq) {
  if (nq <= 0) return 0;
  sskd::Carver c(nullptr);
  c.take<int>((size_t)nq * 11);
  c.take<int>(64);
  c.take<int>(2);
  return c.bytes();
}

int sskd_index_screen_band(const void* d_bf16, int64_t n_rows, const float* d_queries, int nq, float* d_eps2_out,
                           void* d_scratch, size_t scratch_bytes, void* stream) {
  SSKD_REQUIRE(n_rows > 0 && nq > 0, "index_screen_band: needs rows and queries (got rows=%lld nq=%d)", (long long)n_rows, nq);
  int rc = require_shard_rows("index_screen_band", n_rows);
  if (rc != SSKD_OK) return rc;
  SSKD_REQUIRE(d_bf16 && d_queries && d_eps2_out, "index_screen_band: null pointer");
  sskd::Carver c(d_scratch);
  int* const tau = c.take<int>((size_t)nq * 11);
  int* const fb_count = c.take<int>(64);
  int* const status = c.take<int>(2);
  if ((rc = sskd::require_workspace("index_screen_band", d_scratch, scratch_bytes, c.bytes())) != SSKD_OK) return rc;
  const int* max_norm2 = reinterpret_cast<const int*>(static_cast<const char*>(d_bf16) + sidecar_norm_offset(n_rows));
  launch_screen_setup(max_norm2, d_queries, nq, d_eps2_out, tau, fb_count, status, nullptr, 0, sskd::as_stream(stream));
  return sskd::check_launch("screen_setup_kernel");
}

int sskd_index_search_screened_plan(int64_t n_rows, int nq, int k, int* queries_per_block, int* corpus_passes,
                                    int* n_slices) {
  ScreenPlan pl{};
  if (!screen_plan(n_rows, nq, k, &pl)) return sskd::fail(SSKD_ERR_UNSUPPORTED, "index_search_screened_plan: shape not served");
  if (queries_per_block) *queries_per_block = 32 * pl.QB;
  if (corpus_passes) *corpus_passes = pl.n_qblocks;
  if (n_slices) *n_slices = pl.n_slices;
  return SSKD_OK;
}

size_t sskd_index_search_screened_workspace_bytes(int64_t n_rows, int nq, int k) {
  ScreenPlan pl{};
  if (!screen_plan(n_rows, nq, k, &pl)) return 0;
  return screen_carve(nullptr, pl, n_rows, nq, k).bytes;
}

int sskd_index_search_screened(const float* d_tiled, const void* d_bf16, int64_t n_rows, const float* d_queries,
                               int nq, int k, int64_t id_offset, float* d_out_scores, int64_t* d_out_ids,
                               int* d_status, void* d_workspace, size_t workspace_bytes, void* stream,
                               void* ev_scan_begin, void* ev_scan_end) {
  return sskd_index_search_screened_filtered(d_tiled, d_bf16, n_rows, d_queries, nq, k, id_offset, nullptr, d_out_scores,
                                             d_out_ids, d_status, d_workspace, workspace_bytes, stream, ev_scan_begin,
                                             ev_scan_end);
}

int sskd_index_search_screened_filtered(const float* d_tiled, const void* d_bf16, int64_t n_rows, const float* d_queries,
                                        int nq, int k, int64_t id_offset, const uint32_t* d_row_mask, float* d_out_scores,
                                        int64_t* d_out_ids, int* d_status, void* d_workspace, size_t workspace_bytes,
                                        void* stream, void* ev_scan_begin, void* ev_scan_end) {
  return sskd_index_search_screened_claim(d_tiled, d_bf16, n_rows, d_queries, nq, k, id_offset, d_row_mask, -1, d_out_scores,
                                          d_out_ids, d_status, d_workspace, workspace_bytes, stream, ev_scan_begin, ev_scan_end);
}

int sskd_index_search_screened_plan_claims(int64_t n_rows, int nq, int k, int* claims) {
  ScreenPlan pl{};
  if (!screen_plan(n_rows, nq, k, &pl)) return sskd::fail(SSKD_ERR_UNSUPPORTED, "index_search_screened_plan_claims: shape not served");
  if (claims) *claims = pl.claim ? 1 : 0;
  return SSKD_OK;
}

int sskd_index_search_screened_claim(const float* d_tiled, const void* d_bf16, int64_t n_rows, const float* d_queries,
                                     int nq, int k, int64_t id_offset, const uint32_t* d_row_mask, int claim,
                                     float* d_out_scores, int64_t* d_out_ids, int* d_status, void* d_workspace,
                                     size_t workspace_bytes, void* stream, void* ev_scan_begin, void* ev_scan_end) {
  ScreenPlan pl{};
  if (!screen_plan(n_rows, nq, k, &pl))
    return sskd::fail(SSKD_ERR_UNSUPPORTED,
                      "index_search_screened: needs k <= 10, nq >= 64 and >= 2048 rows (got k=%d nq=%d rows=%lld): "
                      "use sskd_index_search", k, nq, (long long)n_rows);
  int rc = require_shard_rows("index_search_screened", n_rows);
  if (rc != SSKD_OK) return rc;
  SSKD_REQUIRE(d_tiled && d_bf16 && d_queries && d_out_scores && d_out_ids && d_status,
               "index_search_screened: null pointer");
  if (claim >= 0) pl.claim = claim != 0;
  const ScreenWs w = screen_carve(d_workspace, pl, n_rows, nq, k);
  if ((rc = sskd::require_workspace("index_search_screened", d_workspace, workspace_bytes, w.bytes)) != SSKD_OK) return rc;
  hipStream_t st = sskd::as_stream(stream);
  const int64_t tiles = sskd::ceil_div(n_rows, TILE_ROWS);
  const int* max_norm2 = reinterpret_cast<const int*>(static_cast<const char*>(d_bf16) + sidecar_norm_offset(n_rows));

  launch_screen_setup(max_norm2, d_queries, nq, w.eps2, w.tau, w.fb_count, d_status, w.cursors, pl.n_qblocks * pl.n_slices, st);

  static_assert((SCREEN_CAP * sizeof(float)) % 256 == 0, "the runs span part_scores and part_ids back to back");
  ScreenAppendParams sp{};
  sp.tiled = static_cast<const sbf16x8*>(d_bf16);
  sp.queries = d_queries;
  sp.eps2 = w.eps2;
  sp.cand = reinterpret_cast<uint2*>(w.part_scores);
  sp.cand_cnt = w.cand_cnt;
  sp.tau = w.tau;
  sp.gpool = w.tau + nq;
  sp.cursors = w.cursors;
  sp.n_rows = n_rows;
  sp.nq = nq;
  sp.lists_per_query = pl.lists_per_query;
  sp.claim = pl.claim ? 1 : 0;
  sp.row_mask = d_row_mask;
#ifdef SSKD_SCREEN_STAMPS
  sp.stamps = w.stamps;
#endif
  const size_t lds = (size_t)pl.QB * BSTEPS * 64 * 16 + (size_t)pl.QB * 32 * 11 * sizeof(int);
  const void* kern = nullptr;
  switch (pl.QB) {
#define SSKD_SCREEN_KERN(qb, light, bg, rg)                                                                           \
  (d_row_mask ? reinterpret_cast<const void*>(screen_append_kernel<10, qb, SCREEN_WAVES, light, bg, rg, true>)       \
              : reinterpret_cast<const void*>(screen_append_kernel<10, qb, SCREEN_WAVES, light, bg, rg>))
#define SSKD_SCREEN_CASE(qb, bg, rg)                                                                                  \
  case qb:                                                                                                            \
    kern = pl.light ? SSKD_SCREEN_KERN(qb, true, bg, rg) : SSKD_SCREEN_KERN(qb, false, bg, rg);                       \
    break;
    SSKD_SCREEN_CASE(2, BGROUP, SCREEN_RING)
    SSKD_SCREEN_CASE(4, BGROUP, SCREEN_RING)
    SSKD_SCREEN_CASE(5, BGROUP_Q5, SCREEN_RING_Q5)
#undef SSKD_SCREEN_CASE
#undef SSKD_SCREEN_KERN
    default:
      return sskd::fail(SSKD_ERR_UNSUPPORTED, "index_search_screened: no screening kernel for %d queries per workgroup", 32 * pl.QB);
  }
  (void)hipFuncSetAttribute(kern, hipFuncAttributeMaxDynamicSharedMemorySize, (int)lds);
  if (ev_scan_begin) (void)hipEventRecord(static_cast<hipEvent_t>(ev_scan_begin), st);
  sp.n_tiles = pl.n_tiles;
  sp.n_slices = pl.n_slices;
  sp.tiles_per_slice = pl.tiles_per_slice;
  sp.pre_tiles = pl.pre_tiles >= SCREEN_WAVES ? pl.pre_tiles : 0;
  sp.pre_tps = sp.pre_tiles ? pl.pre_tps : 0;
  {
    void* args[] = {&sp};
    if (hipLaunchKernel(kern, dim3(pl.n_qblocks * pl.n_slices), dim3(SCREEN_WAVES * 64), args, lds, st) != hipSuccess)
      return sskd::fail(SSKD_ERR_HIP, "index_search_screened: screening launch failed");
  }
  if (ev_scan_end) (void)hipEventRecord(static_cast<hipEvent_t>(ev_scan_end), st);
  rc = sskd::check_launch("screen_append_kernel");
  if (rc != SSKD_OK) return rc;

  ScreenFinalAppendParams fp{};
  fp.cand = sp.cand;
  fp.cand_cnt = w.cand_cnt;
  fp.eps2 = w.eps2;
  fp.rows = d_tiled;
  fp.queries = d_queries;
  fp.lists = pl.lists_per_query;
  fp.k = k;
  fp.nq = nq;
  fp.id_offset = id_offset;
  fp.out_scores = d_out_scores;
  fp.out_ids = d_out_ids;
  fp.fb_count = w.fb_count;
  fp.fb_qid = w.fb_qid;
  fp.fb_queries = w.fb_queries;
  const size_t fin_lds = ((size_t)2 * SCREEN_FIN_ENTRIES + DIM + SCREEN_MAX_CAND) * sizeof(float);
  hipLaunchKernelGGL(screen_finalize_append_kernel, dim3(nq), dim3(64), fin_lds, st, fp);
  if ((rc = sskd::check_launch("screen_finalize_append_kernel")) != SSKD_OK) return rc;

  const int tier1 = nq < SCREEN_FALLBACK_TIER1 ? nq : SCREEN_FALLBACK_TIER1;
  hipLaunchKernelGGL(screen_fallback_tiers_kernel, dim3(1), dim3(1), 0, st, w.fb_count, tier1);
  rc = sskd::exact_search(d_tiled, n_rows, w.fb_queries, tier1, k, id_offset, w.fb_scores, w.fb_ids,
                            w.exact_ws, w.exact_bytes, stream, nullptr, nullptr, nullptr, w.fb_count + 1, d_row_mask);
  if (rc != SSKD_OK) return rc;
  if (nq > tier1) {
    rc = sskd::exact_search(d_tiled, n_rows, w.fb_queries + (size_t)tier1 * DIM, nq - tier1, k, id_offset,
                              w.fb_scores + (size_t)tier1 * k, w.fb_ids + (size_t)tier1 * k, w.exact_ws2, w.exact_bytes2, stream,
                              nullptr, nullptr, nullptr, w.fb_count + 2, d_row_mask);
    if (rc != SSKD_OK) return rc;
  }
  hipLaunchKernelGGL(screen_scatter_kernel, dim3(64), dim3(256), 0, st, w.fb_count, w.fb_qid, w.fb_scores, w.fb_ids, k,
                     d_out_scores, d_out_ids, d_status);
  if ((rc = sskd::check_launch("screen_scatter_kernel")) != SSKD_OK) return rc;
  return SSKD_OK;
}

}
```

Measured before the change: 1.580 million queries/s.

## Switch screening kernel to 16x16x32 bf16 MFMA with packed fp16 thresholds

The bf16 screening kernel moves from 32x32x16 MFMA tiles to pairs of 16x16x32 MFMAs, which changes the corpus and query fragment layouts, the ring and group geometry, and the lane-to-query mapping. Per-query thresholds are now packed two to a register as fp16 and refreshed from LDS only every few tiles, not every tile. The band and the candidate counts move into LDS, and there are four candidate lists per wave instead of two, with a smaller per-list cap. Probe entry points for the scores and the threshold round-trip are added for validation. The aim is lower register pressure and cheaper threshold work per tile, at the cost of more MFMA issues, more LDS traffic, and possible loss of pruning tightness from fp16 rounding of the thresholds.

```diff
diff --git a/include/sskd_amd.h b/include/sskd_amd.h
--- a/include/sskd_amd.h
+++ b/include/sskd_amd.h
@@ -74,6 +74,9 @@
 size_t sskd_index_screen_band_scratch_bytes(int nq);
 int sskd_index_screen_band(const void* d_bf16, int64_t n_rows, const float* d_queries, int nq, float* d_eps2_out,
                            void* d_scratch, size_t scratch_bytes, void* stream);
+
+int sskd_index_screen_scores(const void* d_bf16, int64_t n_rows, const float* d_queries, int nq, float* d_out, void* stream);
+int sskd_screen_threshold_roundtrip(const float* d_in, int n, float* d_out, void* stream);
 
 int sskd_index_search_screened_plan_claims(int64_t n_rows, int nq, int k, int* claims);
 int sskd_index_search_screened_claim(const float* d_tiled, const void* d_bf16, int64_t n_rows, const float* d_queries,
diff --git a/semantic-search-kd_amd/_native.py b/semantic-search-kd_amd/_native.py
--- a/semantic-search-kd_amd/_native.py
+++ b/semantic-search-kd_amd/_native.py
@@ -139,6 +139,8 @@
     ),
     "sskd_index_screen_band_scratch_bytes": (_sz, [_i]),
     "sskd_index_screen_band": (_i, [_vp, _i64, _vp, _i, _vp, _vp, _sz, _vp]),
+    "sskd_index_screen_scores": (_i, [_vp, _i64, _vp, _i, _vp, _vp]),
+    "sskd_screen_threshold_roundtrip": (_i, [_vp, _i, _vp, _vp]),
     "sskd_index_search_onepass_workspace_bytes": (_sz, [_i64, _i, _i]),
     "sskd_index_search_onepass": (_i, [_vp, _i64, _vp, _i, _i, _i64, _vp, _vp, _vp, _vp, _sz, _vp]),
     "sskd_row_mask_words": (_i64, [_i64]),
diff --git a/semantic-search-kd_amd/csrc/screen.hip b/semantic-search-kd_amd/csrc/screen.hip
--- a/semantic-search-kd_amd/csrc/screen.hip
+++ b/semantic-search-kd_amd/csrc/screen.hip
@@ -9,10 +9,11 @@
 namespace {
 
 typedef __bf16 sbf16x8 __attribute__((ext_vector_type(8)));
-constexpr int BSTEPS = DIM / 16;
-constexpr int BTILE_VEC = BSTEPS * 64;
+typedef float f32x4 __attribute__((ext_vector_type(4)));
+constexpr int BSTEPS = DIM / 32;
+constexpr int BTILE_VEC = 2 * BSTEPS * 64;
 #ifndef SSKD_SCREEN_BGROUP
-#define SSKD_SCREEN_BGROUP 6
+#define SSKD_SCREEN_BGROUP 3
 #endif
 #ifndef SSKD_SCREEN_WAVES
 #define SSKD_SCREEN_WAVES 12
@@ -22,11 +23,21 @@
 #endif
 constexpr int BGROUP = SSKD_SCREEN_BGROUP;
 constexpr int SCREEN_RING = SSKD_SCREEN_RING;
-constexpr int BGROUP_Q5 = 3, SCREEN_RING_Q5 = 2;
+#ifndef SSKD_SCREEN_BGROUP_Q5
+#define SSKD_SCREEN_BGROUP_Q5 1
+#endif
+#ifndef SSKD_SCREEN_RING_Q5
+#define SSKD_SCREEN_RING_Q5 3
+#endif
+constexpr int BGROUP_Q5 = SSKD_SCREEN_BGROUP_Q5, SCREEN_RING_Q5 = SSKD_SCREEN_RING_Q5;
 #ifndef SSKD_SCREEN_TAU_REFRESH_TILES
 #define SSKD_SCREEN_TAU_REFRESH_TILES 64
 #endif
 constexpr int SCREEN_TAU_REFRESH_TILES = SSKD_SCREEN_TAU_REFRESH_TILES;
+#ifndef SSKD_SCREEN_BOUND_REFRESH_TILES
+#define SSKD_SCREEN_BOUND_REFRESH_TILES 8
+#endif
+constexpr int SCREEN_BOUND_REFRESH_TILES = SSKD_SCREEN_BOUND_REFRESH_TILES;
 constexpr int SCREEN_WAVES = SSKD_SCREEN_WAVES;
 template <int BG, int RG>
 struct ScreenRingOk {
@@ -162,33 +173,39 @@
 }
 
 template <int BG>
-__device__ __forceinline__ void load_bgroup(sbf16x8 (&buf)[BG], const sbf16x8* __restrict__ base, unsigned lane_off) {
+__device__ __forceinline__ void load_bgroup(sbf16x8 (&buf)[BG][2], const sbf16x8* __restrict__ base, unsigned lane_off) {
   asm volatile("" : "+v"(lane_off));
 #pragma unroll
   for (int s = 0; s < BG; ++s)
-    buf[s] = *reinterpret_cast<const sbf16x8*>(reinterpret_cast<const char*>(base + s * 64) + lane_off);
+#pragma unroll
+    for (int mb = 0; mb < 2; ++mb)
+#ifdef SSKD_SCREEN_ABL_CONTIG
+      buf[s][mb] = *reinterpret_cast<const sbf16x8*>(reinterpret_cast<const char*>(base + s * 128 + mb * 64) + lane_off);
+#else
+      buf[s][mb] = *reinterpret_cast<const sbf16x8*>(reinterpret_cast<const char*>(base + s * 128 + mb * 16) + lane_off);
+#endif
 }
 
 typedef __attribute__((address_space(3))) const sbf16x8 screen_lds_frag;
 constexpr int SCREEN_FRAGS_PER_BASE = 64;
 template <int QB>
-constexpr int screen_frag_bases() { return (QB * BSTEPS + SCREEN_FRAGS_PER_BASE - 1) / SCREEN_FRAGS_PER_BASE; }
+constexpr int screen_frag_bases() { return (2 * QB * BSTEPS + SCREEN_FRAGS_PER_BASE - 1) / SCREEN_FRAGS_PER_BASE; }
 #ifndef SSKD_SCREEN_FRAG_DEPTH
 #define SSKD_SCREEN_FRAG_DEPTH 2
 #endif
 constexpr int SCREEN_FRAG_DEPTH = SSKD_SCREEN_FRAG_DEPTH;
-static_assert(SCREEN_FRAG_DEPTH >= 2, "the fragment ring holds the MFMA's own operand and at least one read ahead");
+static_assert(SCREEN_FRAG_DEPTH >= 2, "the fragment ring holds the MFMAs' own operand and at least one read ahead");
 
 template <int QB, int NB>
 __device__ __forceinline__ sbf16x8 read_qfrag(screen_lds_frag* const (&qbase)[NB], int I) {
-  const int f = (I % QB) * BSTEPS + I / QB;
+  const int f = (I % (2 * QB)) * BSTEPS + I / (2 * QB);
   return qbase[f / SCREEN_FRAGS_PER_BASE][(f % SCREEN_FRAGS_PER_BASE) * 64];
 }
 
 template <int QB, int G, int BG, int D, int NB>
-__device__ __forceinline__ void compute_bgroup(const sbf16x8 (&a)[BG], screen_lds_frag* const (&qbase)[NB], sbf16x8 (&b)[D],
-                                               f32x16 (&acc)[QB]) {
-  constexpr int N = BG * QB, I0 = G * N, TOTAL = BSTEPS * QB;
+__device__ __forceinline__ void compute_bgroup(const sbf16x8 (&a)[BG][2], screen_lds_frag* const (&qbase)[NB], sbf16x8 (&b)[D],
+                                               f32x4 (&acc)[2][2 * QB]) {
+  constexpr int NQ = 2 * QB, N = BG * NQ, I0 = G * N, TOTAL = BSTEPS * NQ;
   asm volatile("" ::: "memory");
 #ifndef SSKD_SCREEN_ABL_NOLDS
   if constexpr (G == 0) {
@@ -198,37 +215,66 @@
 #endif
 #pragma unroll
   for (int i = 0; i < N; ++i) {
-    const int I = I0 + i, s = i / QB, qq = i % QB;
+    const int I = I0 + i, s = i / NQ, nb = i % NQ;
 #ifdef SSKD_SCREEN_ABL_NOLDS
-    const sbf16x8 bi = a[(s + qq) % BG];
+    const sbf16x8 bi = a[(s + nb) % BG][nb & 1];
 #else
     if (I + D - 1 < TOTAL) b[(I + D - 1) % D] = read_qfrag<QB>(qbase, I + D - 1);
     const sbf16x8 bi = b[I % D];
 #endif
     __builtin_amdgcn_sched_barrier(0);
-    acc[qq] = __builtin_amdgcn_mfma_f32_32x32x16_bf16(a[s], bi, acc[qq], 0, 0, 0);
+    acc[0][nb] = __builtin_amdgcn_mfma_f32_16x16x32_bf16(a[s][0], bi, acc[0][nb], 0, 0, 0);
     __builtin_amdgcn_sched_barrier(0);
+    acc[1][nb] = __builtin_amdgcn_mfma_f32_16x16x32_bf16(a[s][1], bi, acc[1][nb], 0, 0, 0);
+    __builtin_amdgcn_sched_barrier(0);
   }
 }
 
 template <int QB, int G, int BG, int RG, int D, int NB>
-__device__ __forceinline__ void screen_tile_groups(sbf16x8 (&buf)[RG][BG], const sbf16x8* __restrict__ tile,
-                                                   screen_lds_frag* const (&qbase)[NB], sbf16x8 (&b)[D], f32x16 (&acc)[QB],
-                                                   bool more, int64_t next_tile, unsigned lane_off) {
+__device__ __forceinline__ void screen_tile_groups(sbf16x8 (&buf)[RG][BG][2], const sbf16x8* __restrict__ tile,
+                                                   screen_lds_frag* const (&qbase)[NB], sbf16x8 (&b)[D],
+                                                   f32x4 (&acc)[2][2 * QB], bool more, int64_t next_tile, unsigned lane_off) {
   constexpr int NG = BSTEPS / BG;
   if constexpr (G < NG) {
     constexpr int PG = G + RG - 1;
 #ifndef SSKD_SCREEN_ABL_NOGLOBAL
-    if constexpr (PG < NG) load_bgroup<BG>(buf[PG % RG], tile + PG * BG * 64, lane_off);
-    else if (more) load_bgroup<BG>(buf[PG % RG], tile + next_tile + (PG - NG) * BG * 64, lane_off);
+    if constexpr (PG < NG) load_bgroup<BG>(buf[PG % RG], tile + PG * BG * 128, lane_off);
+    else if (more) load_bgroup<BG>(buf[PG % RG], tile + next_tile + (PG - NG) * BG * 128, lane_off);
 #endif
     compute_bgroup<QB, G, BG, D, NB>(buf[G % RG], qbase, b, acc);
     screen_tile_groups<QB, G + 1, BG, RG, D, NB>(buf, tile, qbase, b, acc, more, next_tile, lane_off);
   }
 }
 
+typedef _Float16 sf16x2 __attribute__((ext_vector_type(2)));
+__device__ __forceinline__ unsigned screen_thr_pack2(float lo, float hi) {
+  const auto h = __builtin_amdgcn_cvt_pkrtz(lo, hi);
+  unsigned u = __builtin_bit_cast(unsigned, h);
+  u += (float)h[0] > lo ? 1u : 0u;
+  u += (float)h[1] > hi ? 0x10000u : 0u;
+  return u;
+}
+__device__ __forceinline__ float screen_thr_unpack(unsigned packed, int half) {
+  return (float)__builtin_bit_cast(sf16x2, packed)[half];
+}
+#ifndef SSKD_SCREEN_OFFER_SPAN
+#define SSKD_SCREEN_OFFER_SPAN 4
+#endif
+__device__ __forceinline__ float screen_group_max(float x) {
+  if (SSKD_SCREEN_OFFER_SPAN >= 2) x = fmaxf(x, __shfl_xor(x, 16));
+  if (SSKD_SCREEN_OFFER_SPAN >= 4) x = fmaxf(x, __shfl_xor(x, 32));
+  return x;
+}
+__device__ __forceinline__ void screen_thr_raise2(unsigned& packed, float lo, float hi) {
+  const sf16x2 a = __builtin_bit_cast(sf16x2, packed), b = __builtin_bit_cast(sf16x2, screen_thr_pack2(lo, hi));
+  packed = __builtin_bit_cast(unsigned, __builtin_elementwise_max(a, b));
+}
+__device__ __forceinline__ void screen_thr_raise(unsigned& packed, int half, float x) {
+  screen_thr_raise2(packed, half == 0 ? x : -INFINITY, half == 0 ? -INFINITY : x);
+}
+
 #ifndef SSKD_SCREEN_CAP
-#define SSKD_SCREEN_CAP 64
+#define SSKD_SCREEN_CAP 32
 #endif
 #ifndef SSKD_SCREEN_FIN_ENTRIES
 #define SSKD_SCREEN_FIN_ENTRIES 640
@@ -292,13 +338,93 @@
   return w;
 }
 
+template <int QB>
+__device__ __forceinline__ void stage_query_frags(sbf16x8* __restrict__ qs, const float* __restrict__ queries, int q0, int nq,
+                                                  int tid, int n_threads) {
+  for (int idx = tid; idx < 2 * QB * BSTEPS * 64; idx += n_threads) {
+    const int l = idx & 63, sidx = (idx >> 6) % BSTEPS, nb = idx / (64 * BSTEPS);
+    const int q = q0 + nb * 16 + (l & 15);
+    sbf16x8 v;
+#pragma unroll
+    for (int e = 0; e < 8; ++e) v[e] = (__bf16)0.f;
+    if (q < nq) {
+      const float4* src = reinterpret_cast<const float4*>(queries + (int64_t)q * DIM + 32 * sidx + 8 * (l >> 4));
+      const float4 a = src[0], b = src[1];
+      v[0] = (__bf16)a.x; v[1] = (__bf16)a.y; v[2] = (__bf16)a.z; v[3] = (__bf16)a.w;
+      v[4] = (__bf16)b.x; v[5] = (__bf16)b.y; v[6] = (__bf16)b.z; v[7] = (__bf16)b.w;
+    }
+    qs[idx] = v;
+  }
+}
+
+__global__ __launch_bounds__(64) void screen_scores_probe_kernel(const sbf16x8* __restrict__ tiled, const float* __restrict__ queries,
+                                                                 int nq, int n_tiles, float* __restrict__ out) {
+  constexpr int QB = 2, BG = BGROUP, RG = SCREEN_RING, NB = screen_frag_bases<QB>();
+  extern __shared__ float4 qs_raw[];
+  sbf16x8* const qs = reinterpret_cast<sbf16x8*>(qs_raw);
+  const int lane = threadIdx.x, n = lane & 15, g = lane >> 4;
+  stage_query_frags<QB>(qs, queries, 0, nq, lane, 64);
+  __syncthreads();
+  screen_lds_frag* qbase[NB];
+#pragma unroll
+  for (int nb = 0; nb < NB; ++nb) qbase[nb] = (screen_lds_frag*)(qs + lane) + nb * SCREEN_FRAGS_PER_BASE * 64;
+  sbf16x8 buf[RG][BG][2], qfrag[SCREEN_FRAG_DEPTH];
+  const unsigned lane_off = (unsigned)(n + 32 * g) * 16u;
+#pragma unroll
+  for (int gr = 0; gr + 1 < RG; ++gr) load_bgroup<BG>(buf[gr], tiled + gr * BG * 128, lane_off);
+  for (int t = 0; t < n_tiles; ++t) {
+    f32x4 acc[2][2 * QB];
+#pragma unroll
+    for (int mb = 0; mb < 2; ++mb)
+#pragma unroll
+      for (int nb = 0; nb < 2 * QB; ++nb)
+#pragma unroll
+        for (int i = 0; i < 4; ++i) acc[mb][nb][i] = 0.f;
+    screen_tile_groups<QB, 0, BG, RG, SCREEN_FRAG_DEPTH, NB>(buf, tiled + (int64_t)t * BTILE_VEC, qbase, qfrag, acc,
+                                                             t + 1 < n_tiles, (int64_t)BTILE_VEC, lane_off);
+#pragma unroll
+    for (int mb = 0; mb < 2; ++mb)
+#pragma unroll
+      for (int nb = 0; nb < 2 * QB; ++nb)
+#pragma unroll
+        for (int i = 0; i < 4; ++i)
+          out[(int64_t)(t * TILE_ROWS + 16 * mb + 4 * g + i) * (32 * QB) + 16 * nb + n] = acc[mb][nb][i];
+  }
+}
+
+__global__ __launch_bounds__(256) void screen_thr_probe_kernel(const float* __restrict__ in, int n, float* __restrict__ out) {
+  const int i = blockIdx.x * 256 + threadIdx.x;
+  if (i >= n) return;
+  const float x = in[i], y = (i ^ 1) < n ? in[i ^ 1] : -INFINITY;
+  const unsigned packed = (i & 1) ? screen_thr_pack2(y, x) : screen_thr_pack2(x, y);
+  out[i] = screen_thr_unpack(packed, i & 1);
+}
+
+template <int QB>
+__device__ __forceinline__ void apply_tile_mask16(f32x4 (&acc)[2][2 * QB], uint32_t word, int g) {
+  if (word == 0xFFFFFFFFu) return;
+  const uint32_t lw = word >> (4 * g);
+#pragma unroll
+  for (int mb = 0; mb < 2; ++mb)
+#pragma unroll
+    for (int i = 0; i < 4; ++i) {
+      const bool off = ((lw >> (16 * mb + i)) & 1u) == 0u;
+#pragma unroll
+      for (int nb = 0; nb < 2 * QB; ++nb)
+        if (off) acc[mb][nb][i] = -INFINITY;
+    }
+}
+
 template <int K, int QB, int WAVES, bool BOUND_ONLY, bool LIGHT, int BG, int RG, bool MASKED = false>
 __device__ __forceinline__ void screen_tiles(const ScreenAppendParams& p, int t_begin, int t_end, int slice, int* cursors,
-                                             int wave, int j, int h, int q0,
-                                             const sbf16x8* __restrict__ qlane,
-                                             int* __restrict__ pool, int* __restrict__ wthr, uint2* run0, int64_t run_stride,
-                                             bool ragged, float (&gthr)[QB], const float (&band)[QB], int (&cnt)[QB]) {
-  sbf16x8 buf[RG][BG];
+                                             int wave, int n, int g, int q0,
+                                             const sbf16x8* __restrict__ qlane, int* pool, int list0,
+                                             bool ragged, unsigned (&gthr)[QB]) {
+  constexpr int NQ = 2 * QB;
+  int* const wthr = pool + QB * 32 * K;
+  float* const bandl = reinterpret_cast<float*>(wthr + QB * 32);
+  short* const cnts = reinterpret_cast<short*>(bandl + QB * 32);
+  sbf16x8 buf[RG][BG][2];
   constexpr int NB = screen_frag_bases<QB>();
   screen_lds_frag* qbase[NB];
 #pragma unroll
@@ -307,9 +433,11 @@
     asm volatile("" : "+v"(qbase[nb]));
   }
   sbf16x8 qfrag[SCREEN_FRAG_DEPTH];
-  const unsigned lane_off = (unsigned)(j + 32 * h) * 16u;
-  int n_real = p.nq - q0 - j;
-  asm volatile("" : "+v"(n_real));
+#ifdef SSKD_SCREEN_ABL_CONTIG
+  const unsigned lane_off = (unsigned)(n + 16 * g) * 16u;
+#else
+  const unsigned lane_off = (unsigned)(n + 32 * g) * 16u;
+#endif
   constexpr int CH = SCREEN_CLAIM_TILES;
   int t, next_t, c_end = 0, next_end = 0, sl = slice, s_begin = t_begin, s_end = t_end, left = p.n_slices - 1, drawn = 0;
   bool in_flight = false;
@@ -317,7 +445,7 @@
     drawn = 0;
     int at = sl;
     asm volatile("" : "+v"(at));
-    if (j + 32 * h == 0) drawn = __hip_atomic_fetch_add(cursors + at, 1, __ATOMIC_RELAXED, __HIP_MEMORY_SCOPE_AGENT);
+    if (n + 16 * g == 0) drawn = __hip_atomic_fetch_add(cursors + at, 1, __ATOMIC_RELAXED, __HIP_MEMORY_SCOPE_AGENT);
     in_flight = true;
   };
   const auto drawn_chunk = [&]() -> int {
@@ -350,7 +478,7 @@
   }
   if (t >= 0) {
 #pragma unroll
-    for (int g = 0; g + 1 < RG; ++g) load_bgroup<BG>(buf[g], p.tiled + (int64_t)t * BTILE_VEC + g * BG * 64, lane_off);
+    for (int gr = 0; gr + 1 < RG; ++gr) load_bgroup<BG>(buf[gr], p.tiled + (int64_t)t * BTILE_VEC + gr * BG * 128, lane_off);
   }
 
   for (int tiles_done = 0; t >= 0; t = next_t, ++tiles_done) {
@@ -369,119 +497,191 @@
     uint32_t mword = 0xFFFFFFFFu;
     if constexpr (MASKED) mword = tile_mask_word(p.row_mask, t);
     const bool exchange = !BOUND_ONLY && (tiles_done == 0 || tiles_done == 16 || tiles_done % SCREEN_TAU_REFRESH_TILES == 0);
-#pragma unroll
-    for (int qq = 0; qq < QB; ++qq) {
-      const int w = wthr[qq * 32 + j];
-      gthr[qq] = fmaxf(gthr[qq], ordered_to_float(w) - band[qq]);
-      if (exchange && (qq * 32 < n_real))
-        gthr[qq] = fmaxf(gthr[qq],
-                         ordered_to_float(exchange_bound<K>(p.gpool, p.tau + q0 + qq * 32 + j, q0 + qq * 32 + j, w)) - band[qq]);
-    }
-    f32x16 acc[QB];
-#pragma unroll
-    for (int qq = 0; qq < QB; ++qq)
-#pragma unroll
-      for (int r = 0; r < 16; ++r) acc[qq][r] = 0.f;
+    if (exchange || tiles_done % SCREEN_BOUND_REFRESH_TILES == 0) {
+    int nh = n;
+    asm volatile("" : "+v"(nh));
+    if (exchange && g == 0) {
+#pragma unroll
+      for (int nb = 0; nb < NQ; ++nb) {
+        const int ql = 16 * nb + nh;
+        if (q0 + ql < p.nq) atomicMax(wthr + ql, exchange_bound<K>(p.gpool, p.tau + q0 + ql, q0 + ql, wthr[ql]));
+      }
+    }
+#pragma unroll
+    for (int pr = 0; pr < QB; ++pr) {
+      float thr[2];
+#pragma unroll
+      for (int e = 0; e < 2; ++e) {
+        const int nb = 2 * pr + e, ql = 16 * nb + nh;
+        const int w = wthr[ql];
+        const float bd = bandl[ql];
+        thr[e] = ordered_to_float(w) - bd;
+        thr[e] = fmaxf(thr[e], -INFINITY);
+      }
+      screen_thr_raise2(gthr[pr], thr[0], thr[1]);
+      asm volatile("" : "+v"(gthr[pr]));
+    }
+    }
+    f32x4 acc[2][NQ];
+#pragma unroll
+    for (int mb = 0; mb < 2; ++mb)
+#pragma unroll
+      for (int nb = 0; nb < NQ; ++nb)
+#pragma unroll
+        for (int i = 0; i < 4; ++i) acc[mb][nb][i] = 0.f;
 
     screen_tile_groups<QB, 0, BG, RG, SCREEN_FRAG_DEPTH, NB>(buf, tile, qbase, qfrag, acc, next_t >= 0,
                                                              BOUND_ONLY ? (int64_t)WAVES * BTILE_VEC
                                                                         : (int64_t)(next_t - t) * BTILE_VEC, lane_off);
 
-    const int rowbase = t * TILE_ROWS + 4 * h;
+    const int rowbase = t * TILE_ROWS + 4 * g;
     if (ragged && (int64_t)(t + 1) * TILE_ROWS > p.n_rows) {
 #pragma unroll
-      for (int qq = 0; qq < QB; ++qq)
-#pragma unroll
-        for (int r = 0; r < 16; ++r)
-          if (rowbase + acc_row(r) >= p.n_rows) acc[qq][r] = -INFINITY;
-    }
-    if constexpr (MASKED) apply_tile_mask<QB>(acc, mword, h);
+      for (int mb = 0; mb < 2; ++mb)
+#pragma unroll
+        for (int i = 0; i < 4; ++i)
+#pragma unroll
+          for (int nb = 0; nb < NQ; ++nb)
+            if (rowbase + 16 * mb + i >= p.n_rows) acc[mb][nb][i] = -INFINITY;
+    }
+    if constexpr (MASKED) apply_tile_mask16<QB>(acc, mword, g);
 #ifdef SSKD_SCREEN_ABL_NOLIST
 #pragma unroll
-    for (int qq = 0; qq < QB; ++qq)
-#pragma unroll
-      for (int r = 0; r < 16; ++r) asm volatile("" ::"v"(acc[qq][r]));
+    for (int mb = 0; mb < 2; ++mb)
+#pragma unroll
+      for (int nb = 0; nb < NQ; ++nb)
+#pragma unroll
+        for (int i = 0; i < 4; ++i) asm volatile("" ::"v"(acc[mb][nb][i]));
     if (false)
 #endif
 #pragma unroll
-    for (int qq = 0; qq < QB; ++qq) {
-      float m = acc[qq][0];
-#pragma unroll
-      for (int r = 1; r < 16; ++r) m = fmaxf(m, acc[qq][r]);
+    for (int pr = 0; pr < QB; ++pr) {
+      float m[2], fthr[2];
+      bool pass[2];
+#pragma unroll
+      for (int e = 0; e < 2; ++e) {
+        const int nb = 2 * pr + e;
+        m[e] = acc[0][nb][0];
+#pragma unroll
+        for (int r = 1; r < 8; ++r) m[e] = fmaxf(m[e], acc[r >> 2][nb][r & 3]);
+        fthr[e] = fmaxf(screen_thr_unpack(gthr[pr], e), -FLT_MAX);
+        pass[e] = m[e] >= fthr[e];
+      }
       if constexpr (BOUND_ONLY) {
-        if ((qq * 32 < n_real) && m >= gthr[qq]) {
-          int xid = rowbase;
-#pragma unroll
-          for (int r = 15; r >= 0; --r) xid = acc[qq][r] == m ? rowbase + acc_row(r) : xid;
-          const int xi = float_to_ordered(m);
-          if (pool_offer<K>(pool + (qq * 32 + j) * K, wthr + qq * 32 + j, xi)) {
-            int qa = q0 + qq * 32 + j;
-            asm volatile("" : "+v"(qa));
-            bucket_forward<K>(p.gpool, qa, xid, xi);
+#pragma unroll
+        for (int e = 0; e < 2; ++e) {
+          const int nb = 2 * pr + e;
+          const float mg = screen_group_max(pass[e] ? m[e] : -INFINITY);
+          if (pass[e]) {
+            int nc = n;
+            asm volatile("" : "+v"(nc));
+            const int ql = 16 * nb + nc;
+            if (m[e] == mg) {
+              int xid = rowbase;
+#pragma unroll
+              for (int r = 7; r >= 0; --r) xid = acc[r >> 2][nb][r & 3] == m[e] ? rowbase + 16 * (r >> 2) + (r & 3) : xid;
+              const int xi = float_to_ordered(m[e]);
+              if (pool_offer<K>(pool + ql * K, wthr + ql, xi)) {
+                bucket_forward<K>(p.gpool, q0 + ql, xid, xi);
+              }
+            }
+            screen_thr_raise(gthr[pr], e, fmaxf(ordered_to_float(wthr[ql]) - bandl[ql], -INFINITY));
           }
-          gthr[qq] = fmaxf(gthr[qq], ordered_to_float(wthr[qq * 32 + j]) - band[qq]);
         }
       } else
-      if (__any((qq * 32 < n_real) && m >= gthr[qq])) {
+      if (__any(pass[0] || pass[1])) {
+        int nc = n;
+        asm volatile("" : "+v"(nc));
+        float pb[2];
+        int c[2];
+#pragma unroll
+        for (int e = 0; e < 2; ++e) {
+          const int ql = 32 * pr + 16 * e + nc;
+          pb[e] = fmaxf(ordered_to_float(wthr[ql]) - bandl[ql], -INFINITY);
+          c[e] = cnts[(ql * WAVES + wave) * 4 + g];
+        }
+        screen_thr_raise2(gthr[pr], pb[0], pb[1]);
+#pragma unroll
+        for (int e = 0; e < 2; ++e) {
+          const int nb = 2 * pr + e, ql = 16 * nb + nc;
+          const float thr = fmaxf(pb[e], fthr[e]);
+          if (!__any(m[e] >= thr)) continue;
+          short* const cslot = cnts + (ql * WAVES + wave) * 4 + g;
+          unsigned long long* const run = reinterpret_cast<unsigned long long*>(
+              p.cand + ((int64_t)min(q0 + ql, p.nq - 1) * p.lists_per_query + list0 + g) * SCREEN_CAP);
+          int cc = c[e];
+          bool dirty = false;
 #ifndef SSKD_SCREEN_NO_COMPACT
-        {
-          const bool tight = cnt[qq] > SCREEN_CAP - 16 && cnt[qq] <= SCREEN_CAP;
-          if (__any(tight)) {
-            __builtin_amdgcn_s_waitcnt(0x0F70);
-            if (tight) cnt[qq] = screen_compact_run(reinterpret_cast<unsigned long long*>(run0 + qq * run_stride), cnt[qq], gthr[qq]);
+          {
+            const bool tight = cc > SCREEN_CAP - 8 && cc <= SCREEN_CAP;
+            if (__any(tight)) {
+              __builtin_amdgcn_s_waitcnt(0x0F70);
+              if (tight) {
+                cc = screen_compact_run(run, cc, thr);
+                dirty = true;
+              }
+            }
           }
-        }
-#endif
-        bool grew = false;
-#pragma unroll
-        for (int r = 0; r < 16; ++r) {
-          const float x = acc[qq][r];
-          const int xid = rowbase + acc_row(r);
-          const bool take = (qq * 32 < n_real) && x >= gthr[qq];
-          {
-            if (take) {
-              {
-                unsigned long long* const run = reinterpret_cast<unsigned long long*>(run0 + qq * run_stride);
-                if (cnt[qq] < SCREEN_CAP)
-                  run[cnt[qq]] = (unsigned long long)__float_as_uint(x) | ((unsigned long long)(unsigned)xid << 32);
-                ++cnt[qq];
+#endif
+          bool grew = false;
+#pragma unroll
+          for (int r = 0; r < 8; ++r) {
+            const float x = acc[r >> 2][nb][r & 3];
+            const int xid = rowbase + 16 * (r >> 2) + (r & 3);
+            const bool take = x >= thr;
+            {
+              if (take) {
+                {
+                  if (cc < SCREEN_CAP)
+                    run[cc] = (unsigned long long)__float_as_uint(x) | ((unsigned long long)(unsigned)xid << 32);
+                  if (cc <= SCREEN_CAP) ++cc;
+                }
+                if (!LIGHT && tiles_done > 0) {
+                  const int xi = float_to_ordered(x);
+                  if (pool_offer<K>(pool + ql * K, wthr + ql, xi))
+                    bucket_forward<K>(p.gpool, q0 + ql, xid, xi);
+                }
+                grew = true;
               }
-              if (!LIGHT && tiles_done > 0) {
-                const int xi = float_to_ordered(x);
-                if (pool_offer<K>(pool + (qq * 32 + j) * K, wthr + qq * 32 + j, xi) && (qq * 32 < n_real))
-                  bucket_forward<K>(p.gpool, q0 + qq * 32 + j, xid, xi);
-              }
-              grew = true;
+            }
+          }
+          if (grew || dirty) *cslot = (short)cc;
+          const float mg = (LIGHT || tiles_done == 0) ? screen_group_max(m[e]) : m[e];
+          if (grew) {
+            if (m[e] != mg) {
+            } else
+            if constexpr (LIGHT) {
+              int xid = rowbase;
+#pragma unroll
+              for (int r = 7; r >= 0; --r) xid = acc[r >> 2][nb][r & 3] == m[e] ? rowbase + 16 * (r >> 2) + (r & 3) : xid;
+              const int xi = float_to_ordered(m[e]);
+              if (pool_offer<K>(pool + ql * K, wthr + ql, xi) && tiles_done > 0)
+                bucket_forward<K>(p.gpool, q0 + ql, xid, xi);
+            } else {
+              if (tiles_done == 0) pool_offer<K>(pool + ql * K, wthr + ql, float_to_ordered(m[e]));
             }
           }
         }
-        if (grew) {
-          if constexpr (LIGHT) {
-            int xid = rowbase;
-#pragma unroll
-            for (int r = 15; r >= 0; --r) xid = acc[qq][r] == m ? rowbase + acc_row(r) : xid;
-            const int xi = float_to_ordered(m);
-            if (pool_offer<K>(pool + (qq * 32 + j) * K, wthr + qq * 32 + j, xi) && tiles_done > 0)
-              bucket_forward<K>(p.gpool, q0 + qq * 32 + j, xid, xi);
-          } else {
-            if (tiles_done == 0) pool_offer<K>(pool + (qq * 32 + j) * K, wthr + qq * 32 + j, float_to_ordered(m));
-          }
-          gthr[qq] = fmaxf(gthr[qq], ordered_to_float(wthr[qq * 32 + j]) - band[qq]);
-        }
-      }
-    }
-  }
-
-}
+      }
+    }
+  }
+
+}
+
+constexpr size_t screen_lds_bytes(int QB, int WAVES) {
+  return (size_t)2 * QB * BSTEPS * 64 * 16 + (size_t)QB * 32 * (10 + 2) * sizeof(int) + (size_t)QB * 32 * WAVES * 4 * sizeof(short);
+}
+static_assert(screen_lds_bytes(5, SCREEN_WAVES) <= 160 * 1024, "the 160-query workgroup must fit the CU's LDS");
 
 template <int K, int QB, int WAVES, bool LIGHT, int BG, int RG, bool MASKED = false>
 __global__ __launch_bounds__(WAVES * 64) void screen_append_kernel(ScreenAppendParams p) {
+  static_assert(K == 10, "screen_lds_bytes counts ten pool slots per query");
   extern __shared__ float4 qs_raw[];
   sbf16x8* const qs = reinterpret_cast<sbf16x8*>(qs_raw);
   const int tid = threadIdx.x;
   const int lane = tid & 63;
   const int wave = __builtin_amdgcn_readfirstlane(tid >> 6);
-  const int j = lane & 31, h = lane >> 5;
+  const int n = lane & 15, g = lane >> 4;
   const int n_qblocks = gridDim.x / p.n_slices;
   const int xcd = blockIdx.x & 7, within = blockIdx.x >> 3;
   const int logical = xcd * (gridDim.x >> 3) + min(xcd, (int)(gridDim.x & 7)) + within;
@@ -493,41 +693,22 @@
   if (lane == 0) stamp[0] = __builtin_amdgcn_s_memrealtime();
 #endif
 
-  for (int idx = tid; idx < QB * BSTEPS * 64; idx += WAVES * 64) {
-    const int l = idx & 63, sidx = (idx >> 6) % BSTEPS, qq = idx / (64 * BSTEPS);
-    const int q = q0 + qq * 32 + (l & 31);
-    sbf16x8 v;
-#pragma unroll
-    for (int e = 0; e < 8; ++e) v[e] = (__bf16)0.f;
-    if (q < p.nq) {
-      const float4* src = reinterpret_cast<const float4*>(p.queries + (int64_t)q * DIM + 16 * sidx + 8 * (l >> 5));
-      const float4 a = src[0], b = src[1];
-      v[0] = (__bf16)a.x; v[1] = (__bf16)a.y; v[2] = (__bf16)a.z; v[3] = (__bf16)a.w;
-      v[4] = (__bf16)b.x; v[5] = (__bf16)b.y; v[6] = (__bf16)b.z; v[7] = (__bf16)b.w;
-    }
-    qs[idx] = v;
-  }
-  int* const pool = reinterpret_cast<int*>(qs + QB * BSTEPS * 64);
+  stage_query_frags<QB>(qs, p.queries, q0, p.nq, tid, WAVES * 64);
+  int* const pool = reinterpret_cast<int*>(qs + 2 * QB * BSTEPS * 64);
   int* const wthr = pool + QB * 32 * K;
+  float* const bandl = reinterpret_cast<float*>(wthr + QB * 32);
+  short* const cnts = reinterpret_cast<short*>(bandl + QB * 32);
   for (int i = tid; i < QB * 32 * (K + 1); i += WAVES * 64) pool[i] = (int)0x80000000;
+  for (int i = tid; i < QB * 32; i += WAVES * 64) bandl[i] = p.eps2[min(q0 + i, p.nq - 1)];
+  for (int i = tid; i < QB * 32 * WAVES * 2; i += WAVES * 64) reinterpret_cast<int*>(cnts)[i] = 0;
   __syncthreads();
   const sbf16x8* qlane = qs + lane;
 
-  float gthr[QB];
-  float band[QB];
-  int cnt[QB];
-  bool real[QB];
-#pragma unroll
-  for (int qq = 0; qq < QB; ++qq) {
-    gthr[qq] = -FLT_MAX;
-    const int qg = q0 + qq * 32 + j;
-    real[qq] = qg < p.nq;
-    band[qq] = p.eps2[real[qq] ? qg : p.nq - 1];
-    cnt[qq] = 0;
-  }
-  const int my_list = (slice * WAVES + wave) * 2 + h;
-  uint2* const run0 = p.cand + ((int64_t)min(q0 + j, p.nq - 1) * p.lists_per_query + my_list) * SCREEN_CAP;
-  const int64_t run_stride = (int64_t)32 * p.lists_per_query * SCREEN_CAP;
+  unsigned gthr[QB];
+#pragma unroll
+  for (int pr = 0; pr < QB; ++pr)
+    gthr[pr] = (q0 + 32 * pr + n < p.nq ? 0xFC00u : 0x7C00u) | (q0 + 32 * pr + 16 + n < p.nq ? 0xFC000000u : 0x7C000000u);
+  const int list0 = (slice * WAVES + wave) * 4;
 
   const bool ragged = (p.n_rows & 31) != 0;
 
@@ -536,11 +717,11 @@
   if (p.pre_tps > 0) {
     const int s_begin = slice * p.pre_tps;
     const int s_end = min(s_begin + p.pre_tps, p.pre_tiles);
-    screen_tiles<K, QB, WAVES, true, LIGHT, BG, RG, MASKED>(p, s_begin, s_end, slice, nullptr, wave, j, h, q0, qlane,
-                                             pool, wthr, run0, run_stride, ragged, gthr, band, cnt);
-#pragma unroll
-    for (int qq = 0; qq < QB; ++qq)
-      if (real[qq] && h == 0) atomicMax(p.tau + q0 + qq * 32 + j, wthr[qq * 32 + j]);
+    screen_tiles<K, QB, WAVES, true, LIGHT, BG, RG, MASKED>(p, s_begin, s_end, slice, nullptr, wave, n, g, q0, qlane,
+                                             pool, list0, ragged, gthr);
+#pragma unroll
+    for (int nb = 0; nb < 2 * QB; ++nb)
+      if (g == 0 && q0 + nb * 16 + n < p.nq) atomicMax(p.tau + q0 + nb * 16 + n, wthr[nb * 16 + n]);
     __syncthreads();
     if ((SCREEN_STEAL && p.claim) || (s_begin < t_end && t_begin < s_end)) {
       for (int i = tid; i < QB * 32 * K; i += WAVES * 64) pool[i] = (int)0x80000000;
@@ -551,17 +732,17 @@
   if (lane == 0) stamp[1] = __builtin_amdgcn_s_memrealtime();
 #endif
   screen_tiles<K, QB, WAVES, false, LIGHT, BG, RG, MASKED>(p, t_begin, t_end, slice, p.cursors + (int64_t)qblk * p.n_slices,
-                                            wave, j, h, q0, qlane, pool, wthr, run0, run_stride, ragged, gthr, band, cnt);
+                                            wave, n, g, q0, qlane, pool, list0, ragged, gthr);
 #ifdef SSKD_SCREEN_STAMPS
   if (lane == 0) stamp[2] = __builtin_amdgcn_s_memrealtime();
 #endif
 
-  int jt = j;
-  asm volatile("" : "+v"(jt));
-#pragma unroll
-  for (int qq = 0; qq < QB; ++qq) {
-    const int q = q0 + qq * 32 + jt;
-    if (q < p.nq) p.cand_cnt[(int64_t)q * p.lists_per_query + my_list] = cnt[qq];
+  int nt = n;
+  asm volatile("" : "+v"(nt));
+#pragma unroll
+  for (int nb = 0; nb < 2 * QB; ++nb) {
+    const int q = q0 + nb * 16 + nt;
+    if (q < p.nq) p.cand_cnt[(int64_t)q * p.lists_per_query + list0 + g] = cnts[((nb * 16 + nt) * WAVES + wave) * 4 + g];
   }
 }
 
@@ -840,14 +1021,14 @@
   if (pl.QB == 0) return false;
   pl.n_qblocks = (int)sskd::ceil_div(nq, 32 * pl.QB);
   pl.LK = SCREEN_CAP;
-  const int max_by_lists = 1024 / (2 * SCREEN_WAVES);
+  const int max_by_lists = 2048 / (4 * SCREEN_WAVES);
   if (slices > max_by_lists) slices = max_by_lists;
 #ifdef SSKD_SCREEN_FORCE_SLICES
   slices = SSKD_SCREEN_FORCE_SLICES;
 #endif
   pl.tiles_per_slice = (int)sskd::ceil_div(pl.n_tiles, slices);
   pl.n_slices = (int)sskd::ceil_div(pl.n_tiles, pl.tiles_per_slice);
-  pl.lists_per_query = pl.n_slices * SCREEN_WAVES * 2;
+  pl.lists_per_query = pl.n_slices * SCREEN_WAVES * 4;
   pl.part_elems = (size_t)nq * pl.lists_per_query * pl.LK;
   pl.light = pl.tiles_per_slice <= SCREEN_LIGHT_MAX_TILES_PER_WAVE * SCREEN_WAVES;
   pl.claim = pl.tiles_per_slice >= SCREEN_CLAIM_MIN_CHUNKS * SCREEN_WAVES * SCREEN_CLAIM_TILES &&
@@ -964,6 +1145,27 @@
   return sskd::check_launch("screen_setup_kernel");
 }
 
+int sskd_index_screen_scores(const void* d_bf16, int64_t n_rows, const float* d_queries, int nq, float* d_out, void* stream) {
+  SSKD_REQUIRE(n_rows > 0 && nq > 0 && nq <= 64, "index_screen_scores: needs rows and 1..64 queries (got rows=%lld nq=%d)",
+               (long long)n_rows, nq);
+  int rc = require_shard_rows("index_screen_scores", n_rows);
+  if (rc != SSKD_OK) return rc;
+  SSKD_REQUIRE(d_bf16 && d_queries && d_out, "index_screen_scores: null pointer");
+  const size_t lds = (size_t)2 * 2 * BSTEPS * 64 * 16;
+  hipLaunchKernelGGL(screen_scores_probe_kernel, dim3(1), dim3(64), lds, sskd::as_stream(stream),
+                     static_cast<const sbf16x8*>(d_bf16), d_queries, nq, (int)sskd::ceil_div(n_rows, TILE_ROWS), d_out);
+  return sskd::check_launch("screen_scores_probe_kernel");
+}
+
+int sskd_screen_threshold_roundtrip(const float* d_in, int n, float* d_out, void* stream) {
+  SSKD_REQUIRE(n >= 0, "screen_threshold_roundtrip: n < 0");
+  if (n == 0) return SSKD_OK;
+  SSKD_REQUIRE(d_in && d_out, "screen_threshold_roundtrip: null pointer");
+  hipLaunchKernelGGL(screen_thr_probe_kernel, dim3((unsigned)sskd::ceil_div(n, 256)), dim3(256), 0, sskd::as_stream(stream),
+                     d_in, n, d_out);
+  return sskd::check_launch("screen_thr_probe_kernel");
+}
+
 int sskd_index_search_screened_plan(int64_t n_rows, int nq, int k, int* queries_per_block, int* corpus_passes,
                                     int* n_slices) {
   ScreenPlan pl{};
@@ -1026,7 +1228,7 @@
 
   launch_screen_setup(max_norm2, d_queries, nq, w.eps2, w.tau, w.fb_count, d_status, w.cursors, pl.n_qblocks * pl.n_slices, st);
 
-  static_assert((SCREEN_CAP * sizeof(float)) % 256 == 0, "the runs span part_scores and part_ids back to back");
+  static_assert((4 * SCREEN_WAVES * SCREEN_CAP * sizeof(float)) % 256 == 0, "the runs span part_scores and part_ids back to back");
   ScreenAppendParams sp{};
   sp.tiled = static_cast<const sbf16x8*>(d_bf16);
   sp.queries = d_queries;
@@ -1044,7 +1246,7 @@
 #ifdef SSKD_SCREEN_STAMPS
   sp.stamps = w.stamps;
 #endif
-  const size_t lds = (size_t)pl.QB * BSTEPS * 64 * 16 + (size_t)pl.QB * 32 * 11 * sizeof(int);
+  const size_t lds = screen_lds_bytes(pl.QB, SCREEN_WAVES);
   const void* kern = nullptr;
   switch (pl.QB) {
 #define SSKD_SCREEN_KERN(qb, light, bg, rg)                                                                           \
```

Result: faster. 1.700 million queries/s (median of 6 runs) (+7.6%).
